# millecker/hadoop-1.0.3-gpu

Measured on AMD Instinct MI355X. Metric: K-Means job makespan + map-tasks/sec (whole node) at 1/2/4/8 MI355X, higher is better.
Workload: dtype fp32

## Files before the change

### hbmr/models/kmeans.py

```python
from __future__ import annotations

import base64
import logging
import math
import os
import threading
import time

import numpy as np
import torch

from ..gpu.splitjob import SplitJob, SplitSpec
from ..mapred import counters as C

log = logging.getLogger("hbmr.kmeans")

K_KEY = "hbmr.kmeans.k"
D_KEY = "hbmr.kmeans.dims"
INPUT_KEY = "hbmr.kmeans.input"
SPLIT_PTS_KEY = "hbmr.split.points"
CIN_KEY = "hbmr.kmeans.centroids.in"
COUT_KEY = "hbmr.kmeans.centroids.out"
INIT_KEY = "hbmr.kmeans.centroids.init"
NCENTERS_KEY = "hbmr.kmeans.synthetic.centers"
RETURN_KEY = "hbmr.kmeans.return.centroids"
CDIR_KEY = "hbmr.kmeans.centroids.dir"
EXACT_KEY = "hbmr.kmeans.exact"
EXACT_MFMA_KEY = "hbmr.kmeans.exact.mfma"
COMBINER_KEY = "hbmr.kmeans.combiner"
BOUNDS_KEY = "hbmr.kmeans.exact.bounds"

_M32 = 0xFFFFFFFF


def _mix32(x: torch.Tensor) -> torch.Tensor:
    x = x & _M32
    x = ((x ^ (x >> 16)) * 0x45D9F3B) & _M32
    x = ((x ^ (x >> 16)) * 0x45D9F3B) & _M32
    return x ^ (x >> 16)


def _uniform(c: torch.Tensor) -> torch.Tensor:
    return (_mix32(c).to(torch.float64) + 0.5) * (1.0 / 4294967296.0)


def _gauss(c1: torch.Tensor, c2: torch.Tensor) -> torch.Tensor:
    u1 = _uniform(c1)
    u2 = _uniform(c2)
    return torch.sqrt(-2.0 * torch.log(u1)) * torch.cos(2.0 * math.pi * u2)


def synthetic_points(seed: int, start: int, n: int, d: int, centers: int, device,
                     chunk: int = 1 << 18) -> torch.Tensor:
    dev = torch.device(device)
    out = torch.empty(n, d, dtype=torch.float32, device=dev)
    j = torch.arange(d, dtype=torch.int64, device=dev)
    cidx = torch.arange(centers, dtype=torch.int64, device=dev)
    s = (seed * 0x9E3779B1) & _M32
    cc = (cidx[:, None] * 131071 + j[None, :] + s * 7) & _M32
    cen = 10.0 * _gauss(cc * 2 + 1, cc * 2 + 2)
    for a in range(0, n, chunk):
        b = min(n, a + chunk)
        p = torch.arange(start + a, start + b, dtype=torch.int64, device=dev)
        lab = _mix32(p * 3 + s) % centers
        base = ((p[:, None] & 0xFFFFFF) * 1024 + j[None, :] + (s << 7)) & _M32
        noise = _gauss(base * 2 + 11, base * 2 + 12 + (p[:, None] >> 24))
        out[a:b] = (cen[lab] + noise).to(torch.float32)
    return out


def encode_centroids(c: torch.Tensor) -> str:
    a = c.detach().to("cpu", torch.float32).contiguous().numpy()
    return f"{a.shape[0]}x{a.shape[1]}:" + base64.b64encode(a.tobytes()).decode()


def decode_centroids(s: str) -> torch.Tensor:
    shp, b = s.split(":", 1)
    k, d = map(int, shp.split("x"))
    return torch.from_numpy(np.frombuffer(base64.b64decode(b), dtype=np.float32).copy()
                            ).reshape(k, d)


class CentroidStore:

    def __init__(self):
        self.lock = threading.Lock()
        self.host: dict[str, torch.Tensor] = {}
        self.images: dict[tuple, object] = {}
        self.order: list[str] = []
        self.keep = 4

    def put_host(self, key, cen):
        with self.lock:
            self.host[key] = cen
            for k in [k for k in self.images if k[0] == key]:
                self.images.pop(k)
            self._touch(key)

    def put_image(self, key, device, img):
        with self.lock:
            self.host.pop(key, None)
            self.images[(key, str(device))] = img
            self._touch(key)

    def _touch(self, key):
        if key in self.order:
            self.order.remove(key)
        self.order.append(key)
        while len(self.order) > self.keep:
            old = self.order.pop(0)
            self.host.pop(old, None)
            for k in [k for k in self.images if k[0] == old]:
                self.images.pop(k)
# ... 93 lines not shown
_BASELINES: "dict" = {}
_BASE_LOCK = threading.Lock()
_BASE_MAX = 4096


def _baseline_plan(ctxs, datas, k, dp, fx, exact, enabled):
    have, new, plain = [], [], []
    bases, keys = [], []
    seen = set()
    dev = str(ctxs[0].device)
    with _BASE_LOCK:
        for i, (c, d) in enumerate(zip(ctxs, datas)):
            sp = c.spec.split
            sk = sp.get("key") if enabled and isinstance(sp, dict) else None
            key = None if sk is None else (sk, dev, k, dp, fx, exact)
            keys.append(key)
            if key is None or key in seen:
                plain.append(i)
                bases.append(None)
                continue
            seen.add(key)
            b = _BASELINES.get(key)
            x = d.xb if exact else d
            if b is not None and b.data_ptr == x.data_ptr() and b.n == x.shape[0]:
                have.append(i)
                bases.append(b)
            else:
                new.append(i)
                bases.append(None)
    return have, new, plain, bases, keys


def _baseline_bytes(b) -> int:
    return sum(t.numel() * t.element_size() for t in (b.g, b.S0, b.N0, getattr(b, "gap", None))
               if t is not None)


def _drop_baselines(split_key, device):
    dev = f"cuda:{device}" if isinstance(device, int) else str(device)
    with _BASE_LOCK:
        for key in [kk for kk in _BASELINES if kk[0] == split_key and kk[1] == dev]:
            _BASELINES.pop(key)


def _install_baselines(entries, stream, cache=None, grown=None):
    ev = torch.cuda.Event()
    ev.record(stream)
    charge = []
    with _BASE_LOCK:
        for key, b in entries:
            b.event, b.stream = ev, stream
            old = _BASELINES.pop(key, None)
            _BASELINES[key] = b
            if old is not b:
                charge.append((key, b, _baseline_bytes(b)))
            elif grown and grown.get(id(b)):
                charge.append((key, b, grown[id(b)]))
        while len(_BASELINES) > _BASE_MAX:
            _BASELINES.pop(next(iter(_BASELINES)))
    if cache is not None and charge:
        cache.add_listener(_drop_baselines)
        idx = stream.device.index if stream is not None else 0
        for key, b, nbytes in charge:
            if not cache.charge(key[0], idx, nbytes):
                with _BASE_LOCK:
                    if _BASELINES.get(key) is b:
                        _BASELINES.pop(key)


def _exact_stats(cin, device):
    key = (cin, str(device))
    with _EXACT_LOCK:
        t = _EXACT_STATS.get(key)
        if t is None:
            t = _EXACT_STATS[key] = torch.zeros(3, dtype=torch.int64, device=device)
        return t


def _exact_skipped(cin, device):
    key = (cin, str(device))
    with _EXACT_LOCK:
        t = _EXACT_SKIPPED.get(key)
        if t is None:
            t = _EXACT_SKIPPED[key] = torch.zeros(1, dtype=torch.int64, device=device)
        return t


class KMeansSplitJob(SplitJob):
    collective_reduce = True
    needs_reduce = True

    def configure(self, conf):
        self.conf = conf
        self.k = conf.get_int(K_KEY, 64)
        self.d = conf.get_int(D_KEY, 128)
        self.input = conf.get(INPUT_KEY, "synthetic:100000:1")
        self.split_points = conf.get_int(SPLIT_PTS_KEY, 500_000)
        self.cin = conf.get(CIN_KEY)
        self.cout = conf.get(COUT_KEY)
        self.centers = conf.get_int(NCENTERS_KEY, self.k)
        self.fx_shift = conf.get_int("hbmr.kmeans.fx.shift", 24)
        self.cdir = conf.get(CDIR_KEY)
        self.exact = conf.get_boolean(EXACT_KEY, False)
        self.exact_dtype = torch.bfloat16 if (conf.get(EXACT_MFMA_KEY) or "f16").lower() in (
            "bf16", "bfloat16") else torch.float16
        self.bounds = conf.get_boolean(BOUNDS_KEY, True)
        self.combiner = (conf.get(COMBINER_KEY) or "delta").lower()
        if self.combiner not in ("delta", "sorted"):
            raise ValueError(f"{COMBINER_KEY} must be delta or sorted, not {self.combiner!r}")
        init = conf.get(INIT_KEY)
        if init and self.cin and STORE.host_centroids(self.cin) is None:
            STORE.put_host(self.cin, decode_centroids(init))
        if self.cin and self.cdir and STORE.host_centroids(self.cin) is None:
            path = _centroid_file(self.cdir, self.cin)
            if os.path.exists(path):
                STORE.put_host(self.cin, torch.from_numpy(np.load(path)))

    _split_memo: dict = {}

    def get_splits(self, conf, trackers):
        if self.input.startswith("synthetic:"):
            mk = (self.input, self.split_points, self.d, self.centers, tuple(trackers),
                  self.exact)
            got = KMeansSplitJob._split_memo.get(mk)
            if got is not None:
                return got
            if len(KMeansSplitJob._split_memo) > 16:
                KMeansSplitJob._split_memo.clear()
            out = KMeansSplitJob._split_memo[mk] = self._synthetic_splits(trackers)
            return out
        return self._file_splits(conf, trackers)

    def _synthetic_splits(self, trackers):
        _, n, seed = self.input.split(":")
        n, seed = int(n), int(seed)
        per = self.split_points
        nsplits = max(1, math.ceil(n / per))
        out = []
        for i in range(nsplits):
            a = i * per
            m = min(per, n - a)
            key = f"kmeans-syn:{seed}:{self.d}:{self.centers}:{a}:{m}" + \
                (":exact" if self.exact else "")
            loc = [trackers[i * len(trackers) // nsplits]] if trackers else []
            out.append(SplitSpec(i, key, "synthetic",
                                 {"seed": seed, "start": a, "n": m}, loc, m * self.d * 2))
        return out

    def _file_splits(self, conf, trackers):
        from ..mapred.formats import FileInputFormat, SequenceFileInputFormat
        from ..mapred.jobconf import JobConf
        jc = JobConf(conf)
        FileInputFormat.setInputPaths(jc, self.input)
        fmt = SequenceFileInputFormat()
        nmaps = max(1, conf.get_int("mapred.map.tasks", 1))
        if conf.get_long("mapred.min.split.size", 0) <= 1 and "://" not in self.input:
            total = sum(f.length for f in fmt.list_status(jc))
            jc.set_long("mapred.min.split.size", max(1, -(-total // nmaps)))
        splits = fmt.getSplits(jc, nmaps)
        out = []
        for i, s in enumerate(splits):
            key = f"kmeans-file:{s.path}:{s.start}:{s.length}" + (":exact" if self.exact else "")
            loc = [trackers[i % len(trackers)]] if trackers else []
            out.append(SplitSpec(i, key, "file", {"path": s.path, "start": s.start,
                                                  "length": s.length}, loc, s.length))
        return out

    def _load_raw(self, spec: SplitSpec, device):
        if spec.kind == "synthetic":
            p = spec.params
            return synthetic_points(p["seed"], p["start"], p["n"], self.d, self.centers, device)
        return self._load_file_split(spec.params, device)

    def _load_fp32(self, spec: SplitSpec, device):
        return self._load_raw(spec, device).to(torch.bfloat16)

    def split_nbytes(self, data) -> int:
        nb = getattr(data, "nbytes", None)
        if callable(nb):
            return int(nb())
        return super().split_nbytes(data)

    def load_split_host(self, spec: SplitSpec):
        if spec.kind != "file":
            return None
        from ..io import nativeio
        p = spec.params
        n = p["length"] // (20 + 4 * self.d) + 2
        host = torch.empty(n, self.d, dtype=torch.float32,
# ... 92 lines not shown
    def _map_gpu_batch(self, ctxs, datas):
        from ..ops import kmeans as km
        ctx = ctxs[0]
        img = STORE.image(self.cin, ctx.device)
        ready = getattr(img, "ready", None)
        if ready is not None:
            torch.cuda.current_stream().wait_event(ready)
        for t in (img.cbf, img.chalf):
            t.record_stream(torch.cuda.current_stream())
        B = len(datas)
        if self.exact:
            return self._map_exact(ctxs, datas, img)
        have, new, plain, bases, keys = _baseline_plan(
            ctxs, datas, self.k, img.dp, img.fx_shift, False, self.combiner == "delta")
        ws, labels = self._scratch(ctx, [d.shape[0] for d in datas], self.k)
        sums = torch.empty(B, self.k, img.dp, dtype=torch.int64, device=ctx.device)
        counts = torch.empty(B, self.k, dtype=torch.int64, device=ctx.device)
        order = have + new + plain
        H = len(have)
        S, N = sums.unbind(0), counts.unbind(0)
        out = [None] * B
        for j, i in enumerate(order):
            out[i] = (S[j], N[j])
        installed = []
        if have:
            hb = [bases[i] for i in have]
            km.map_batch_delta([datas[i] for i in have], img, sums[:H], counts[:H], labels, ws,
                               hb, stream=ctx.stream)
            for i, b in zip(have, hb):
                b.S0, b.N0 = out[i]
                installed.append((keys[i], b))
        rest = new + plain
        if rest:
            km.map_batch_gpu([datas[i] for i in rest], img, sums[H:], counts[H:], labels, ws,
                             stream=ctx.stream, zero_outputs=True)
            if new:
                total = sum(datas[i].shape[0] for i in rest)
                gall = labels[:total].clone()
                off = 0
                newset = set(new)
                for i in rest:
                    n = datas[i].shape[0]
                    if keys[i] is not None and i in newset:
                        installed.append((keys[i], km.Baseline(gall[off:off + n], *out[i],
                                                                datas[i].data_ptr(), n)))
                    off += n
        if installed:
            _install_baselines(installed, ctx.stream, getattr(ctx, "split_cache", None))
        for c, d in zip(ctxs, datas):
            c.reporter.incrCounter(C.TASK_GROUP, C.MAP_INPUT_RECORDS, d.shape[0])
        return out

    def _map_exact(self, ctxs, datas, img):
        from ..ops import kmeans as km
        from ..utils.trace import TRACE
        if TRACE.on:
            TRACE.instant("kmeans.map_exact", n=len(datas))
        ctx = ctxs[0]
        store = ctx.tracker.__dict__.setdefault("_scratch", {})
        scratch = store.setdefault(("kmeans-exact", str(ctx.device), id(ctx.stream)), {})
        stats = _exact_stats(self.cin, ctx.device)
        have, new, plain, bases, keys = _baseline_plan(
            ctxs, datas, self.k, img.dp, img.fx_shift, True, self.combiner == "delta")
        B = len(datas)
        sums = torch.empty(B, self.k, img.dp, dtype=torch.int64, device=ctx.device)
        counts = torch.empty(B, self.k, dtype=torch.int64, device=ctx.device)
        order = have + new + plain
        pos = {i: j for j, i in enumerate(order)}
        H = len(have)
        installed = []
        grown = None
        if have:
            ns = [datas[i].shape[0] for i in have]
            total = sum(ns)
            lab = scratch.get("labcat")
            if lab is None or lab.numel() < total:
                lab = scratch["labcat"] = torch.empty(total, dtype=torch.int32, device=ctx.device)
            need = km.delta_workspace_bytes(total, H, self.k)
            if scratch.get("dws") is None or scratch["dws"].numel() < need:
                scratch["dws"] = torch.empty(need, dtype=torch.uint8, device=ctx.device)
            hb = [bases[i] for i in have]
            bounded = self.bounds and self.combiner == "delta" and km.bounds_supported(img)
            if bounded:
                nogap = [b for b in hb if b.gap is None]
                km.assign_exact_batch([datas[i] for i in have], img, stats, lab, scratch,
                                      stream=ctx.stream, bounds=hb,
                                      skipped=_exact_skipped(self.cin, ctx.device))
                grown = {id(b): b.gap.numel() * b.gap.element_size() for b in nogap}
            else:
                km.assign_exact_batch([datas[i] for i in have], img, stats, lab, scratch,
                                      stream=ctx.stream)
            km.delta_combine([datas[i].x32 for i in have], lab, self.k, sums[:H], counts[:H],
                             scratch["dws"], hb, fx_shift=img.fx_shift, stream=ctx.stream,
                             keep_bounds=bounded)
            for i, b in zip(have, hb):
                b.S0, b.N0 = sums[pos[i]], counts[pos[i]]
                installed.append((keys[i], b))
        for i in new + plain:
            d = datas[i]
            s, c = sums[pos[i]], counts[pos[i]]
            s.zero_()
            c.zero_()
            lab = km.assign_exact(d, img, stats, scratch, stream=ctx.stream)
            need = km.workspace_bytes(d.shape[0], img.k)
            if scratch.get("ws") is None or scratch["ws"].numel() < need:
                scratch["ws"] = torch.empty(max(need, 1 << 20), dtype=torch.uint8,
                                            device=ctx.device)
            km.accumulate(d.x32, lab, img.k, s, c, fx_shift=img.fx_shift, stream=ctx.stream,
                          workspace=scratch["ws"])
            if keys[i] is not None and i in new:
                b = km.Baseline(lab.clone(), s, c, d.xb.data_ptr(), d.shape[0])
                installed.append((keys[i], b))
        if installed:
            _install_baselines(installed, ctx.stream, getattr(ctx, "split_cache", None), grown)
        for c, d in zip(ctxs, datas):
            c.reporter.incrCounter(C.TASK_GROUP, C.MAP_INPUT_RECORDS, d.shape[0])
        return [(sums[pos[i]], counts[pos[i]]) for i in range(B)]

    def map_cpu(self, ctx, points):
        from ..ops import kmeans as km
        cen = STORE.host_centroids(self.cin)
        if cen is None:
            raise KeyError(f"centroids {self.cin!r} not resident")
        sums, counts = km.new_partials(self.k, self.d, "cpu")
        st = [0]
        km.map_split_cpu(points, cen, sums, counts, nthreads=ctx.cpu_threads,
                         fx_shift=self.fx_shift, exact=self.exact, stats=st)
        if self.exact:
            ctx.reporter.incrCounter("KMEANS", "EXACT_FLAGGED_POINTS", st[0])
        ctx.reporter.incrCounter(C.TASK_GROUP, C.MAP_INPUT_RECORDS, points.shape[0])
        return sums, counts

    def map_sim(self, ctx, points):
        if points is None:
            ctx.reporter.incrCounter(C.TASK_GROUP, C.MAP_INPUT_RECORDS, 0)
            return None
        return self.map_cpu(ctx, points)

    def combine(self, ctx, outputs):
        from ..ops import kmeans as km
        dev = ctx.device if ctx.device is not None else torch.device("cpu")
        dp = km.padded_dim(self.d) if dev.type == "cuda" else self.d
        outputs = [o for o in outputs if o is not None]
        if dev.type == "cuda":
            cur = torch.cuda.current_stream()
            for s, c in outputs:
                if s.is_cuda:
                    s.record_stream(cur)
                    c.record_stream(cur)
        from ..utils.trace import TRACE
        if TRACE.on:
            TRACE.instant("kmeans.combine.recorded", n=len(outputs))
        same = [(s, c) for s, c in outputs if s.device == dev and s.shape[1] == dp]
        other = [(s, c) for s, c in outputs if not (s.device == dev and s.shape[1] == dp)]
        if same:
            sums, counts = _sum_slabs(same)
        else:
            sums = torch.zeros(self.k, dp, dtype=torch.int64, device=dev)
            counts = torch.zeros(self.k, dtype=torch.int64, device=dev)
        for s, c in other:
            sums[:, :s.shape[1]] += s.to(dev, non_blocking=True)
            counts += c.to(dev, non_blocking=True)
        return sums, counts

    def reduce(self, ctx, combined):
        from ..ops import kmeans as km
        from ..utils.trace import TRACE
        sums, counts = combined
        k, dp = sums.shape
        packed = torch.cat([sums.reshape(-1), counts])
        sim = getattr(ctx, "simulated_collective_s", None)
        with TRACE.span("kmeans.allreduce", nbytes=packed.numel() * 8):
            if sim is None:
                ctx.comm.all_reduce(packed)
            else:
                ctx.sim_ready = max(time.time(), getattr(ctx, "sim_base", 0.0)) + sim
        sums = packed[:k * dp].view(k, dp)
        counts = packed[k * dp:]
        est = _EXACT_STATS.pop((self.cin, str(sums.device)), None) \
            if self.exact and sums.device.type == "cuda" else None
        esk = _EXACT_SKIPPED.pop((self.cin, str(sums.device)), None) \
            if self.exact and sums.device.type == "cuda" else None
        killed = getattr(ctx, "killed", None)
        if killed is not None and killed():
            raise RuntimeError("reduce killed (collective restart): result not published")
        if sums.device.type == "cuda":
            old = STORE.image(self.cin, sums.device)
            ready = getattr(old, "ready", None)
            if ready is not None:
                torch.cuda.current_stream().wait_event(ready)
            img = km.CentroidImage.__new__(km.CentroidImage)
            img.__dict__.update(old.__dict__)
            img.cen = old.cen.clone()
            img.cbf = old.cbf.clone()
            img.chalf = old.chalf.clone()
            img.shift2 = torch.zeros_like(old.shift2)
            img.refresh(sums, counts)
            if self.exact:
                img.image16(self.exact_dtype)
                img.neighbors()
            img.ready = torch.cuda.Event()
            img.ready.record()
            host_cen = cen_ev = None
            if ctx.rank == 0 and (self.cdir or self.conf.get_boolean(RETURN_KEY, False)):
                host_cen = torch.empty(tuple(img.cen.shape), dtype=torch.float32,
                                       pin_memory=True)
                host_cen.copy_(img.cen, non_blocking=True)
                cen_ev = torch.cuda.Event()
                cen_ev.record()
            if TRACE.on:
                TRACE.instant("kmeans.refresh_launched")
            STORE.put_image(self.cout, sums.device, img)
            rel = getattr(ctx, "release_dependents", None)
            if rel is not None:
                rel()
            vals = [img.shift2.max().double().sqrt(), counts.sum().double()]
            if est is not None:
                vals += list(est.double().unbind(0))
            if esk is not None:
                vals.append(esk[0].double())
            got = torch.stack(vals).tolist()
            shift, npts = got[0], got[1]
            if esk is not None:
                ctx.reporter.incrCounter("KMEANS", "EXACT_BOUND_SKIPPED_POINTS", int(got[-1]))
            if est is not None:
                for name, v in zip(("EXACT_FLAGGED_POINTS", "EXACT_RELABELLED_POINTS",
                                    "EXACT_NEIGHBOUR_SCANS"), got[2:5]):
                    ctx.reporter.incrCounter("KMEANS", name, int(v))
            if TRACE.on:
                TRACE.instant("kmeans.shift_synced")
            new_cen = None
        else:
            host_cen = cen_ev = None
            old = STORE.host_centroids(self.cin)
            if sim is not None:
                new_cen, shift, npts = old, 0.0, 0
            else:
                cnt = counts.to(torch.float64)[:, None]
                s = sums[:, :self.d].to(torch.float64) / float(1 << self.fx_shift)
                new_cen = torch.where(cnt > 0, s / cnt.clamp(min=1),
                                      old.to(torch.float64)).to(torch.float32)
                shift = float((new_cen - old).norm(dim=1).max()) if self.k else 0.0
                npts = int(counts.sum().item())
            STORE.put_host(self.cout, new_cen)
            rel = getattr(ctx, "release_dependents", None)
            if rel is not None:
                rel()
            if sim is not None:
                delay = ctx.sim_ready - time.time()
                if delay > 0:
                    time.sleep(delay)
        self._write_output(ctx, counts, new_cen)
        if TRACE.on:
            TRACE.instant("kmeans.output_written")
        res = {"shift": shift, "points": int(npts), "centroids_key": self.cout}
        if host_cen is not None:
            cen_ev.synchronize()
        if ctx.rank == 0 and self.cdir:
            cen = new_cen if new_cen is not None else host_cen
            _save_centroids(self.cdir, self.cout, cen[:, :self.d])
        if ctx.rank == 0 and self.conf.get_boolean(RETURN_KEY, False):
            cen = new_cen if new_cen is not None else host_cen
            res["centroids"] = encode_centroids(cen[:, :self.d])
        if TRACE.on:
            TRACE.instant("kmeans.reduce_return")
        return res

    def poison_result(self, ctx):
        with STORE.lock:
            host = STORE.host.get(self.cout)
            if host is not None:
                STORE.host[self.cout] = host + 1.0
            for key, img in list(STORE.images.items()):
                if key[0] == self.cout:
                    STORE.images.pop(key)
                    STORE.host[self.cout] = img.cen.detach().to("cpu")[:, :self.d] + 1.0

    def _write_output(self, ctx, counts, new_cen):
        out = self.conf.get("mapred.output.dir")
        if not out:
            return
        import os

        from ..io import sequencefile as seqf
        from ..io.writable import FloatVectorWritable, IntWritable
        cen = new_cen if new_cen is not None else STORE.host_centroids(self.cout)
        W = ctx.world_size
        per = math.ceil(self.k / W)
        lo, hi = ctx.rank * per, min(self.k, (ctx.rank + 1) * per)
        os.makedirs(out, exist_ok=True)
        with seqf.Writer(os.path.join(out, f"part-{ctx.rank:05d}"), IntWritable,
                         FloatVectorWritable) as w:
            for j in range(lo, hi):
                w.append(IntWritable(j), FloatVectorWritable(cen[j].numpy()))


def make_iteration_conf(base, k, d, inp, split_points, cin, cout, init=None,
                        return_centroids=False):
    from ..mapred.jobconf import JobConf
    job = JobConf(base)
    job.set_job_name(f"kmeans {cin}->{cout}")
    job.set("hbmr.splitjob.class", "hbmr.models.kmeans:KMeansSplitJob")
    job.set("hbmr.gpu.mapper.class", "hbmr.models.kmeans:KMeansSplitJob")
    job.set_int(K_KEY, k)
    job.set_int(D_KEY, d)
    job.set(INPUT_KEY, inp)
    job.set_int(SPLIT_PTS_KEY, split_points)
# ... 189 lines not shown
```

### hbmr/ops/_lib.py

```python
from __future__ import annotations

import ctypes
import os
import threading
from pathlib import Path

import torch

_LIB_PATH = Path(__file__).resolve().parent.parent / "lib" / "libhbmr.so"
_lock = threading.Lock()
_lib = None

c_void_p = ctypes.c_void_p
c_long = ctypes.c_long
c_int = ctypes.c_int
c_uint = ctypes.c_uint
c_uint64 = ctypes.c_uint64
c_double_p = ctypes.POINTER(ctypes.c_double)

_SIGS = {
    "hbmr_kmeans_assign_bf16": (c_int, [c_void_p, c_long, c_int, c_void_p, c_void_p, c_int,
                                        c_void_p, c_void_p, c_void_p]),
    "hbmr_kmeans_accum_bf16": (c_int, [c_void_p, c_long, c_int, c_void_p, c_int, c_void_p,
                                       c_void_p, c_int, c_void_p, c_long, c_int, c_void_p]),
    "hbmr_kmeans_accum_f32": (c_int, [c_void_p, c_long, c_int, c_void_p, c_int, c_void_p,
                                      c_void_p, c_int, c_void_p, c_long, c_int, c_void_p]),
    "hbmr_kmeans_assign_top3_bf16": (c_int, [c_void_p, c_long, c_int, c_void_p, c_void_p, c_int,
                                             c_void_p, c_void_p, c_void_p, c_void_p, c_void_p]),
    "hbmr_kmeans_assign_top3_f16": (c_int, [c_void_p, c_long, c_int, c_void_p, c_void_p, c_int,
                                            c_void_p, c_void_p, c_void_p, c_void_p, c_void_p]),
    "hbmr_kmeans_exact_prep": (c_int, [c_void_p, c_long, c_int, c_int, c_int, c_int, c_void_p,
                                       c_void_p, c_void_p, c_void_p, c_void_p]),
    "hbmr_kmeans_assign_top3_q1_grouped": (c_int, [c_int, c_void_p, c_void_p, c_int, c_int,
                                                   c_void_p, c_void_p, c_void_p, c_int, c_void_p,
                                                   c_void_p, c_void_p, c_void_p, c_int, c_int,
                                                   c_void_p, c_void_p, c_void_p, c_void_p,
                                                   c_void_p, c_long, c_void_p, c_void_p]),
    "hbmr_kmeans_bound_workspace_bytes": (c_long, [c_long, c_int, c_int]),
    "hbmr_kmeans_assign_top3_q1_bounded": (c_int, [c_int, c_void_p, c_void_p, c_int, c_int,
                                                   c_void_p, c_void_p, c_int, c_void_p,
                                                   c_void_p, c_void_p, c_void_p, c_int, c_int,
                                                   c_void_p, c_void_p, c_void_p, c_void_p,
                                                   c_void_p, c_long, c_void_p,
                                                   c_void_p, c_void_p, c_void_p, c_void_p,
                                                   c_void_p, c_long, c_void_p, c_void_p]),
    "hbmr_kmeans_centroid_nbr": (c_int, [c_void_p, c_int, c_int, c_int, c_void_p, c_void_p,
                                         c_void_p, c_void_p]),
    "hbmr_kmeans_image16": (c_int, [c_void_p, c_int, c_int, c_int, c_int, c_int, c_void_p,
                                    c_void_p, c_void_p, c_void_p, c_void_p, c_void_p]),
    "hbmr_kmeans_image16_tiled": (c_int, [c_void_p, c_int, c_int, c_void_p, c_void_p]),
    "hbmr_kmeans_set_exact_kernel": (c_int, [c_int]),
    "hbmr_kmeans_get_exact_kernel": (c_int, []),
    "hbmr_kmeans_refine_f32": (c_int, [c_void_p, c_long, c_int, c_int, c_void_p, c_void_p,
                                       c_void_p, c_void_p, c_int, c_int, c_void_p, c_void_p,
                                       c_void_p, c_void_p, c_void_p, c_void_p, c_int, c_void_p,
                                       c_void_p, c_void_p, c_void_p, c_void_p, c_int,
                                       c_void_p]),
    "hbmr_kmeans_refine_batch_bytes": (c_long, [c_int, c_void_p]),
    "hbmr_kmeans_assign_top3_grouped": (c_int, [c_int, c_void_p, c_void_p, c_int, c_int,
                                                c_void_p, c_void_p, c_int, c_void_p, c_void_p,
                                                c_void_p, c_void_p, c_void_p]),
    "hbmr_kmeans_refine_batch_q1g": (c_int, [c_int, c_void_p, c_int, c_int, c_int, c_void_p,
                                             c_void_p, c_void_p, c_void_p, c_void_p, c_void_p,
                                             c_void_p, c_void_p, c_void_p, c_void_p, c_void_p,
                                             c_void_p, c_long, c_void_p, c_void_p]),
    "hbmr_kmeans_refine_batch_q1": (c_int, [c_int, c_void_p, c_int, c_int, c_int, c_int,
                                            c_void_p, c_void_p, c_void_p, c_void_p, c_void_p,
                                            c_void_p, c_void_p, c_void_p, c_void_p, c_void_p,
                                            c_void_p, c_void_p, c_void_p, c_long, c_int,
                                            c_void_p, c_void_p]),
    "hbmr_kmeans_refine_batch_finish": (c_int, [c_int, c_void_p, c_void_p, c_void_p, c_int,
                                                c_int, c_void_p, c_int, c_int, c_void_p,
                                                c_void_p, c_void_p, c_void_p, c_int, c_void_p,
                                                c_int, c_void_p, c_long, c_void_p]),
    "hbmr_kmeans_accum_workspace_bytes": (c_long, [c_long, c_int]),
    "hbmr_kmeans_batch_workspace_bytes": (c_long, [c_long, c_int, c_int]),
    "hbmr_kmeans_map_batch": (c_int, [c_int, c_void_p, c_void_p, c_int, c_void_p, c_void_p, c_int,
                                      c_int, c_void_p, c_void_p, c_long, c_void_p, c_void_p,
                                      c_int, c_int, c_void_p]),
    "hbmr_kmeans_delta_workspace_bytes": (c_long, [c_long, c_int, c_int]),
    "hbmr_kmeans_delta_combine": (c_int, [c_int, c_void_p, c_void_p, c_int, c_int, c_int,
                                          c_void_p, c_void_p, c_long, c_void_p, c_void_p, c_int,
                                          c_void_p, c_void_p, c_void_p, c_void_p]),
    "hbmr_kmeans_map_batch_delta": (c_int, [c_int, c_void_p, c_void_p, c_int, c_void_p, c_void_p,
                                            c_int, c_int, c_void_p, c_void_p, c_long, c_void_p,
                                            c_void_p, c_int, c_void_p, c_void_p, c_void_p,
                                            c_void_p]),
    "hbmr_kmeans_update": (c_int, [c_void_p, c_void_p, c_int, c_int, c_int, c_int, c_int,
                                   c_void_p, c_void_p, c_void_p, c_void_p, c_void_p]),
    "hbmr_kmeans_padded_k": (c_int, [c_int]),
    "hbmr_kmeans_map_cpu_f32": (c_int, [c_void_p, c_long, c_int, c_void_p, c_int, c_void_p,
                                        c_void_p, c_void_p, c_double_p, c_int, c_int]),
    "hbmr_kmeans_map_cpu_f32_ex": (c_int, [c_void_p, c_long, c_int, c_void_p, c_int, c_void_p,
                                           c_void_p, c_void_p, c_double_p, c_int, c_int, c_int,
                                           c_void_p]),
    "hbmr_kmeans_padded_dim": (c_int, [c_int]),
    "hbmr_f32_to_bf16_pad": (c_int, [c_void_p, c_long, c_int, c_int, c_void_p, c_void_p]),
    "hbmr_radix_sort_workspace_bytes": (c_long, [c_long]),
    "hbmr_radix_onesweep_workspace_bytes": (c_long, [c_long]),
    "hbmr_radix_onesweep_status_bytes": (c_long, [c_long]),
    "hbmr_radix_sort_keys_u64": (c_int, [c_void_p, c_void_p, c_long, c_int, c_int, c_void_p,
                                         c_long, c_void_p, c_long, c_void_p, c_void_p, c_int,
                                         c_void_p]),
    "hbmr_radix_sort_pairs_u64": (c_int, [c_void_p, c_void_p, c_void_p, c_void_p, c_long, c_int,
                                          c_int, c_void_p, c_long, c_void_p]),
    "hbmr_teragen": (c_int, [c_long, c_long, c_void_p, c_void_p]),
    "hbmr_tera_keys": (c_int, [c_void_p, c_long, c_int, c_void_p, c_void_p, c_void_p]),
    "hbmr_gather_u64": (c_int, [c_void_p, c_void_p, c_long, c_void_p, c_void_p]),
    "hbmr_gather_records": (c_int, [c_void_p, c_void_p, c_long, c_int, c_void_p, c_void_p]),
    "hbmr_split_offsets": (c_int, [c_void_p, c_void_p, c_long, c_void_p, c_void_p, c_int,
                                   c_void_p, c_void_p]),
    "hbmr_check_sorted": (c_int, [c_void_p, c_void_p, c_long, c_void_p, c_void_p]),
    "hbmr_tera_keys_part": (c_int, [c_void_p, c_long, c_int, c_void_p, c_void_p, c_int, c_void_p,
                                    c_void_p, c_void_p, c_void_p]),
    "hbmr_tera_collect": (c_int, [c_void_p, c_void_p, c_void_p, c_void_p, c_void_p, c_int, c_long,
                                  c_void_p, c_void_p, c_void_p, c_void_p, c_void_p]),
    "hbmr_tera_collect_slots": (c_int, [c_void_p, c_void_p, c_void_p, c_int, c_int, c_long,
                                        c_void_p, c_void_p, c_void_p]),
    "hbmr_gather_records_multi": (c_int, [c_void_p, c_void_p, c_void_p, c_void_p, c_long, c_int,
                                          c_void_p, c_void_p]),
    "hbmr_tera_partition_workspace_bytes": (c_long, [c_long, c_int]),
    "hbmr_tera_collect_gid": (c_int, [c_void_p, c_void_p, c_void_p, c_void_p, c_int, c_long,
                                      c_int, c_uint64, c_uint, c_uint, c_int, c_void_p, c_void_p,
                                      c_void_p]),
    "hbmr_gather_records_gid": (c_int, [c_void_p, c_void_p, c_void_p, c_long, c_int, c_void_p,
                                        c_void_p, c_void_p, c_void_p, c_void_p]),
    "hbmr_tera_group_stats": (c_int, [c_void_p, c_void_p, c_long, c_void_p, c_void_p, c_void_p,
                                      c_void_p]),
    "hbmr_radix_set_onesweep_waves": (c_int, [c_int]),
    "hbmr_gather_set_unroll": (c_int, [c_int]),
    "hbmr_tera_tie_fix_scratch_bytes": (c_long, [c_long, c_int]),
    "hbmr_tera_tie_fix_records": (c_int, [c_void_p, c_void_p, c_void_p, c_long, c_int, c_uint64,
                                          c_uint, c_uint, c_int, c_void_p, c_void_p, c_void_p,
                                          c_long, c_void_p]),
    "hbmr_merge_path": (c_int, [c_void_p, c_void_p, c_void_p, c_long, c_void_p, c_void_p, c_void_p,
                                c_long, c_void_p, c_void_p, c_void_p, c_void_p]),
    "hbmr_tera_tie_fix": (c_int, [c_void_p, c_void_p, c_void_p, c_long, c_void_p, c_void_p]),
    "hbmr_tera_partition": (c_int, [c_void_p, c_long, c_int, c_void_p, c_void_p, c_int, c_void_p,
                                    c_void_p, c_void_p, c_void_p, c_void_p, c_void_p, c_long,
                                    c_void_p]),
    "hbmr_wc_tiles": (c_long, [c_long]),
    "hbmr_wc_tokenize_count": (c_int, [c_void_p, c_long, c_void_p, c_void_p]),
    "hbmr_wc_tokenize_write": (c_int, [c_void_p, c_long, c_void_p, c_void_p, c_void_p, c_void_p]),
    "hbmr_wc_insert": (c_int, [c_void_p, c_long, c_void_p, c_void_p, c_void_p, c_long, c_void_p,
                               c_void_p, c_long, c_void_p, c_void_p]),
    "hbmr_wc_compact": (c_int, [c_void_p, c_long, c_void_p, c_void_p, c_long, c_int, c_void_p,
                                c_void_p, c_void_p, c_void_p, c_void_p, c_void_p]),
    "hbmr_wc_pack": (c_int, [c_void_p, c_void_p, c_void_p, c_void_p, c_long, c_void_p, c_void_p,
                             c_void_p]),
    "hbmr_grep_cand_count": (c_int, [c_void_p, c_long, c_void_p, c_void_p, c_int, c_int, c_int,
                                     c_int, c_void_p, c_void_p, c_void_p]),
    "hbmr_grep_cand_write": (c_int, [c_void_p, c_long, c_void_p, c_void_p, c_int, c_int, c_int,
                                     c_int, c_void_p, c_void_p, c_void_p, c_void_p, c_void_p]),
    "hbmr_grep_select_blocks": (c_long, [c_long]),
    "hbmr_grep_block_max": (c_int, [c_void_p, c_long, c_void_p, c_void_p]),
    "hbmr_grep_prefix_max": (c_int, [c_void_p, c_long, c_void_p, c_void_p, c_void_p]),
    "hbmr_grep_select_count": (c_int, [c_void_p, c_void_p, c_void_p, c_long, c_void_p, c_void_p]),
# ... 88 lines not shown
```

### hbmr/ops/kmeans.py

```python
from __future__ import annotations

import ctypes
import os
import threading

import torch

from . import _lib
from ..utils.trace import TRACE

SUPPORTED_DP = (64, 128, 256)


def _nullctx():
    import contextlib
    return contextlib.nullcontext()
FX_SHIFT = 24
NBR_L = 256


def padded_dim(d: int) -> int:
    for dp in SUPPORTED_DP:
        if d <= dp:
            return dp
# ... 236 lines not shown
            _lib.check(rc, "hbmr_kmeans_exact_prep")
            return
        x64 = self.x32.double()
        self.xnorm = x64.norm(dim=1).float()
        lim = 65504.0 if dtype == torch.float16 else float("inf")
        xb = self.x32.clamp(-lim, lim).to(dtype)
        xb64 = xb.double()
        self.xbn2 = xb64.pow(2).sum(1).float()
        self.xerr = _f32_up((x64 - xb64).norm(dim=1))
        self.xb = xb.contiguous()

    @property
    def shape(self):
        return self.xb.shape

    def nbytes(self) -> int:
        return sum(t.numel() * t.element_size() for t in (self.xb, self.x32, self.xnorm,
                                                          self.xbn2, self.xerr))


def assign_top3(points: torch.Tensor, img: CentroidImage, labels, cand, scores, margin,
                stream=None) -> None:
    n, dp = points.shape
    if points.dtype not in (torch.bfloat16, torch.float16) or dp != img.dp or \
            not points.is_contiguous():
        raise ValueError("points must be contiguous bf16/fp16 [n, dp] matching the image")
    for t, dt, m in ((labels, torch.int32, 1), (cand, torch.int32, 2), (scores, torch.float32, 1),
                     (margin, torch.float32, 2)):
        if t.numel() != m * n or t.dtype != dt or not t.is_contiguous():
            raise ValueError("top-3 outputs: labels/scores [n], cand/margin [2n]")
    f16 = points.dtype == torch.float16
    with torch.cuda.stream(stream) if stream is not None else _nullctx():
        c16, ch = img.image16(points.dtype)[:2]
    fn = "hbmr_kmeans_assign_top3_f16" if f16 else "hbmr_kmeans_assign_top3_bf16"
    rc = getattr(_lib.load(), fn)(
        _ptr(points), n, dp, _ptr(c16), _ptr(ch), img.k_pad, _ptr(labels),
        _ptr(cand), _ptr(scores), _ptr(margin), _lib.stream_handle(stream))
    _lib.check(rc, fn)


REFINE_VERSION = int(os.environ.get("HBMR_REFINE", "3"))
MAX_REFINE_BATCH = 64


def _refine_ws(ns: list, device, scratch: dict | None):
    arr = (ctypes.c_long * len(ns))(*ns)
    need = int(_lib.load().hbmr_kmeans_refine_batch_bytes(len(ns), arr))
    if need < 0:
        raise ValueError("refine batch of 1..64 splits expected")
    ws = None if scratch is None else scratch.get("refine_ws")
    if ws is None or ws.numel() < need:
        ws = torch.empty(need, dtype=torch.uint8, device=device)
        if scratch is not None:
            scratch["refine_ws"] = ws
    return arr, ws


class _RefineBatch:

    def __init__(self, splits: list, img: "CentroidImage", stats, scratch, stream):
        self.splits, self.img, self.stats, self.stream = splits, img, stats, stream
        self.dt = splits[0].xb.dtype
        self.ns, self.ws = _refine_ws([sp.shape[0] for sp in splits], splits[0].x32.device,
                                      scratch)
        with torch.cuda.stream(stream) if stream is not None else _nullctx():
            self.norms = img.norms(self.dt)
            self.nbr = img.neighbors()
            self.pd = img.pair_dist()
        self.labels = [None] * len(splits)
        self.lib = _lib.load()
        self.st = _lib.stream_handle(stream)

    def q1(self, i, labels_ptr, cand, scores, margin):
        sp, img = self.splits[i], self.img
        cn, cmax, ce, cemax = self.norms
        self.labels[i] = labels_ptr
        rc = self.lib.hbmr_kmeans_refine_batch_q1(
            len(self.splits), self.ns, i, img.d, img.k, img.k_pad, _ptr(sp.xnorm),
            _ptr(sp.xbn2), _ptr(sp.xerr), _ptr(cn), _ptr(cmax), _ptr(ce), _ptr(cemax),
            labels_ptr, _ptr(cand), _ptr(scores), _ptr(margin), _ptr(self.stats),
            _ptr(self.ws), self.ws.numel(), int(i == 0), _ptr(self.pd), self.st)
        _lib.check(rc, "hbmr_kmeans_refine_batch_q1")

    def finish(self):
        B = len(self.splits)
        img = self.img
        _, cmax, _, cemax = self.norms
        ni, nd, L = self.nbr
        xs = (ctypes.c_void_p * B)(*[sp.x32.data_ptr() for sp in self.splits])
        ls = (ctypes.c_void_p * B)(*[(lp.value if isinstance(lp, ctypes.c_void_p) else lp)
                                     for lp in self.labels])
        rc = self.lib.hbmr_kmeans_refine_batch_finish(
            B, self.ns, xs, ls, img.d, self.splits[0].x32.shape[1], _ptr(img.cen), img.k,
            img.k_pad, _ptr(cmax), _ptr(cemax), _ptr(ni), _ptr(nd), L, _ptr(self.stats),
            self.stats.numel(), _ptr(self.ws), self.ws.numel(), self.st)
        _lib.check(rc, "hbmr_kmeans_refine_batch_finish")


def refine_f32(split: ExactSplit, img: CentroidImage, labels, cand, scores, margin,
               stats: torch.Tensor, stream=None, scratch: dict | None = None) -> None:
    n = split.shape[0]
    if stats.dtype != torch.int64 or stats.numel() < 3:
        raise ValueError("stats must be int64 [3]")
    if labels.numel() != n or cand.numel() != 2 * n or margin.numel() != 2 * n:
        raise ValueError("labels [n], cand/margin [2n] from assign_top3 expected")
    if REFINE_VERSION >= 3:
        rb = _RefineBatch([split], img, stats, scratch, stream)
        rb.q1(0, labels.data_ptr(), cand, scores, margin)
        rb.finish()
        return
    with torch.cuda.stream(stream) if stream is not None else _nullctx():
        cn, cmax, ce, cemax = img.norms(split.xb.dtype)
        ni, nd, L = img.neighbors()
    rc = _lib.load().hbmr_kmeans_refine_f32(
        _ptr(split.x32), n, img.d, split.x32.shape[1], _ptr(split.xnorm), _ptr(split.xbn2),
        _ptr(split.xerr), _ptr(img.cen), img.k, img.k_pad, _ptr(cn), _ptr(cmax), _ptr(ce),
        _ptr(cemax), _ptr(ni), _ptr(nd), L,
        _ptr(labels), _ptr(cand), _ptr(scores), _ptr(margin), _ptr(stats), stats.numel(),
        _lib.stream_handle(stream))
    _lib.check(rc, "hbmr_kmeans_refine_f32")


def assign_exact(split: ExactSplit, img: CentroidImage, stats: torch.Tensor,
                 scratch: dict | None = None, stream=None) -> torch.Tensor:
    n = split.shape[0]
    dev = split.xb.device
    scratch = {} if scratch is None else scratch
    key = ("exact", n)
    bufs = scratch.get(key)
    if bufs is None:
        bufs = scratch[key] = (torch.empty(n, dtype=torch.int32, device=dev),
                               torch.empty(2 * n, dtype=torch.int32, device=dev),
                               torch.empty(n, dtype=torch.float32, device=dev),
                               torch.empty(2 * n, dtype=torch.float32, device=dev))
    lab, cand, sc, mg = bufs
    assign_top3(split.xb, img, lab, cand, sc, mg, stream=stream)
    refine_f32(split, img, lab, cand, sc, mg, stats, stream=stream, scratch=scratch)
    return lab


def bounds_supported(img: CentroidImage) -> bool:
    return REFINE_VERSION >= 3 and img.dp <= 128 and GROUPED_EXACT and FUSED_Q1 and \
        img.cen.is_cuda and _lib.load().hbmr_kmeans_get_exact_kernel() == 3


def assign_exact_batch(splits: list, img: CentroidImage, stats: torch.Tensor, out: torch.Tensor,
                       scratch: dict | None = None, stream=None, bounds: list | None = None,
                       skipped: torch.Tensor | None = None) -> None:
    if not splits:
        return
    if bounds is not None and (len(bounds) != len(splits) or not bounds_supported(img)):
        raise ValueError("bounds: one baseline per split, grouped fused v3 assign (dp <= 128)")
    dev = splits[0].xb.device
    total = sum(sp.shape[0] for sp in splits)
    if out.dtype != torch.int32 or out.numel() < total or not out.is_contiguous():
        raise ValueError("out must be contiguous int32 with room for every split's labels")
    if stats.dtype != torch.int64 or stats.numel() < 3:
        raise ValueError("stats must be int64 [3]")
    dt = splits[0].xb.dtype
    for sp in splits:
        if sp.xb.dtype != dt or dt not in (torch.bfloat16, torch.float16) or \
                sp.xb.shape[1] != img.dp or not sp.xb.is_contiguous() or \
                not sp.x32.is_contiguous():
            raise ValueError("exact splits must hold contiguous [n, dp] rows of one 16-bit type")
    nmax = max(sp.shape[0] for sp in splits)
    scratch = {} if scratch is None else scratch
    key = ("exact-batch", nmax)
    bufs = scratch.get(key)
    if bufs is None:
        for kk in [kk for kk in scratch if isinstance(kk, tuple) and kk[0] == "exact-batch"]:
            del scratch[kk]
        bufs = scratch[key] = (torch.empty(2 * nmax, dtype=torch.int32, device=dev),
                               torch.empty(nmax, dtype=torch.float32, device=dev),
                               torch.empty(2 * nmax, dtype=torch.float32, device=dev))
    cand, sc, mg = bufs
    grouped = REFINE_VERSION >= 3 and img.dp <= 128 and GROUPED_EXACT
    with torch.cuda.stream(stream) if stream is not None else _nullctx():
        c16, ch, cn, cmax, ce, cemax = img.image16(dt)
        ni, nd, L = (None, None, 0) if grouped else img.neighbors()
        newref = None
        if bounds is not None:
            img.cen.record_stream(torch.cuda.current_stream())
            newref = img.cen.clone()
    lib = _lib.load()
    top3 = lib.hbmr_kmeans_assign_top3_f16 if dt == torch.float16 else \
        lib.hbmr_kmeans_assign_top3_bf16
    st = _lib.stream_handle(stream)
    pc, ps, pm, pst = _ptr(cand), _ptr(sc), _ptr(mg), _ptr(stats)
    pcn, pcmax, pce, pcemax, pni, pnd = (_ptr(t) for t in (cn, cmax, ce, cemax, ni, nd))
    base, off = out.data_ptr(), 0
    for g0 in range(0, len(splits), MAX_REFINE_BATCH):
        group = splits[g0:g0 + MAX_REFINE_BATCH]
        if grouped:
            off += _exact_group(group, img, stats, base + 4 * off, c16, ch, (cn, cmax, ce, cemax),
                                dt, scratch, stream, lib, st,
                                None if bounds is None else bounds[g0:g0 + MAX_REFINE_BATCH],
                                skipped, newref)
            continue
        rb = _RefineBatch(group, img, stats, scratch, stream) if REFINE_VERSION >= 3 else None
        for i, sp in enumerate(group):
            n = sp.shape[0]
            pl = ctypes.c_void_p(base + 4 * off)
            rc = top3(_ptr(sp.xb), n, img.dp, _ptr(c16), _ptr(ch), img.k_pad, pl, pc, ps, pm, st)
            _lib.check(rc, "hbmr_kmeans_assign_top3")
            if rb is not None:
                rb.q1(i, pl, cand, sc, mg)
            else:
                rc = lib.hbmr_kmeans_refine_f32(
                    _ptr(sp.x32), n, img.d, sp.x32.shape[1], _ptr(sp.xnorm), _ptr(sp.xbn2),
                    _ptr(sp.xerr), _ptr(img.cen), img.k, img.k_pad, pcn, pcmax, pce, pcemax,
                    pni, pnd, L, pl, pc, ps, pm, pst, stats.numel(), st)
                _lib.check(rc, "hbmr_kmeans_refine_f32")
            off += n
        if rb is not None:
            rb.finish()


PAIR_DIST_MAX_K = int(os.environ.get("HBMR_PAIR_DIST_MAX_K", "8192"))
NBR_NATIVE_MAX_K = int(os.environ.get("HBMR_NBR_NATIVE_MAX_K", "8192"))
GROUPED_EXACT = os.environ.get("HBMR_EXACT_GROUPED", "1") != "0"
FUSED_Q1 = os.environ.get("HBMR_EXACT_FUSED_Q1", "1") != "0"


def _bounded_group(group, bases, img, labels_ptr, ch, norms, dt, scratch, stream, lib, st, rb,
                   skipped, newref):
    B = len(group)
    ns = [sp.shape[0] for sp in group]
    N = sum(ns)
    dev = group[0].xb.device
    cur = torch.cuda.current_stream() if stream is None else stream
    with torch.cuda.stream(cur):
        events, blocks = {}, {}
        for b in bases:
            if b.event is not None and b.stream is not None and b.stream != cur:
                events[id(b.event)] = b.event
        for ev in events.values():
            cur.wait_event(ev)
        for b in bases:
            if b.gap is None:
                b.gap, b.ref = torch.empty(b.g.numel(), dtype=torch.float32, device=dev), None
        for b, n in zip(bases, ns):
            if b.g.numel() != n or b.gap.numel() != n or \
                    (b.ref is not None and (tuple(b.ref.shape) != tuple(img.cen.shape) or
                                            not b.ref.is_contiguous())):
                raise ValueError("bounds: baseline does not match its split / the centroids")
            for t in (b.g, b.gap, b.ref):
                if t is not None:
                    base = t._base if t._base is not None else t
                    blocks[id(base)] = base
        for t in blocks.values():
            t.record_stream(cur)
        need = int(lib.hbmr_kmeans_bound_workspace_bytes(N, B, img.k))
        bws = scratch.get("bound_ws")
        if bws is None or bws.numel() < need:
            bws = scratch["bound_ws"] = torch.empty(need, dtype=torch.uint8, device=dev)
    P = ctypes.c_void_p * B
    cn, cmax, ce, cemax = norms
    refs = [b.ref for b in bases]
    for b in bases:
        b.ref = b.pending = None
    rc = lib.hbmr_kmeans_assign_top3_q1_bounded(
        B, P(*[sp.xb.data_ptr() for sp in group]), (ctypes.c_long * B)(*ns), img.dp,
        int(dt == torch.float16), _ptr(img.image16_tiled(dt)), _ptr(ch), img.k_pad, labels_ptr,
        P(*[sp.xnorm.data_ptr() for sp in group]), P(*[sp.xbn2.data_ptr() for sp in group]),
        P(*[sp.xerr.data_ptr() for sp in group]), img.d, img.k, _ptr(cn), _ptr(cmax), _ptr(ce),
        _ptr(cemax), _ptr(rb.ws), rb.ws.numel(), _ptr(rb.pd),
        P(*[b.g.data_ptr() for b in bases]), P(*[b.gap.data_ptr() for b in bases]),
        P(*[None if r is None else r.data_ptr() for r in refs]), _ptr(img.cen),
        _ptr(bws), bws.numel(), _ptr(skipped), st)
    _lib.check(rc, "hbmr_kmeans_assign_top3_q1_bounded")
    for b in bases:
        b.pending = newref


def _exact_group(group, img, stats, labels_ptr, c16, ch, norms, dt, scratch, stream, lib, st,
                 bases=None, skipped=None, newref=None):
    B = len(group)
    ns = [sp.shape[0] for sp in group]
    N = sum(ns)
    dev = group[0].xb.device
    P = ctypes.c_void_p * B
    xs = P(*[sp.xb.data_ptr() for sp in group])
    nsa = (ctypes.c_long * B)(*ns)
    if bases is not None:
        rb = _RefineBatch(group, img, stats, scratch, stream)
        if TRACE.on:
            TRACE.instant("kmeans.top3_launch", n=B)
        _bounded_group(group, bases, img, labels_ptr, ch, norms, dt, scratch, stream, lib, st, rb,
                       skipped, newref)
        o = 0
        for i in range(B):
            rb.labels[i] = labels_ptr + 4 * o
            o += ns[i]
        rb.finish()
        return N
    if FUSED_Q1 and img.dp <= 128:
        rb = _RefineBatch(group, img, stats, scratch, stream)
        if TRACE.on:
            TRACE.instant("kmeans.top3_launch", n=B)
        cn, cmax, ce, cemax = norms
        rc = lib.hbmr_kmeans_assign_top3_q1_grouped(
            B, xs, nsa, img.dp, int(dt == torch.float16), _ptr(c16),
            _ptr(img.image16_tiled(dt)), _ptr(ch), img.k_pad,
            labels_ptr, P(*[sp.xnorm.data_ptr() for sp in group]),
            P(*[sp.xbn2.data_ptr() for sp in group]), P(*[sp.xerr.data_ptr() for sp in group]),
            img.d, img.k, _ptr(cn), _ptr(cmax), _ptr(ce), _ptr(cemax), _ptr(rb.ws),
            rb.ws.numel(), _ptr(rb.pd), st)
        _lib.check(rc, "hbmr_kmeans_assign_top3_q1_grouped")
        o = 0
        for i in range(B):
            rb.labels[i] = labels_ptr + 4 * o
            o += ns[i]
        rb.finish()
        return N
    key = ("exact-group", N)
    bufs = scratch.get(key)
    if bufs is None:
        for kk in [kk for kk in scratch if isinstance(kk, tuple) and kk[0] == "exact-group"]:
            del scratch[kk]
        bufs = scratch[key] = (torch.empty(2 * N, dtype=torch.int32, device=dev),
                               torch.empty(N, dtype=torch.float32, device=dev),
                               torch.empty(2 * N, dtype=torch.float32, device=dev))
    cand, sc, mg = bufs
    rc = lib.hbmr_kmeans_assign_top3_grouped(B, xs, nsa, img.dp, int(dt == torch.float16),
                                             _ptr(c16), _ptr(ch), img.k_pad, labels_ptr,
                                             _ptr(cand), _ptr(sc), _ptr(mg), st)
    _lib.check(rc, "hbmr_kmeans_assign_top3_grouped")
    rb = _RefineBatch(group, img, stats, scratch, stream)
    cn, cmax, ce, cemax = norms
    rc = lib.hbmr_kmeans_refine_batch_q1g(
        B, nsa, img.d, img.k, img.k_pad, P(*[sp.xnorm.data_ptr() for sp in group]),
        P(*[sp.xbn2.data_ptr() for sp in group]), P(*[sp.xerr.data_ptr() for sp in group]),
        _ptr(cn), _ptr(cmax), _ptr(ce), _ptr(cemax), labels_ptr, _ptr(cand), _ptr(sc), _ptr(mg),
        _ptr(rb.ws), rb.ws.numel(), _ptr(rb.pd), st)
    _lib.check(rc, "hbmr_kmeans_refine_batch_q1g")
    o = 0
    for i in range(B):
        rb.labels[i] = labels_ptr + 4 * o
        o += ns[i]
    rb.finish()
    return N


def map_split_exact(split: ExactSplit, img: CentroidImage, sums, counts, scratch: dict,
                    stats: torch.Tensor, stream=None) -> None:
    n = split.shape[0]
    lab = assign_exact(split, img, stats, scratch, stream=stream)
    need = workspace_bytes(n, img.k)
    if scratch.get("ws") is None or scratch["ws"].numel() < need:
        scratch["ws"] = torch.empty(max(need, 1 << 20), dtype=torch.uint8, device=split.xb.device)
    accumulate(split.x32, lab, img.k, sums, counts, fx_shift=img.fx_shift, stream=stream,
               workspace=scratch["ws"])


def map_batch_gpu(splits: list, img: CentroidImage, sums: torch.Tensor, counts: torch.Tensor,
                  labels: torch.Tensor, workspace: torch.Tensor, stream=None,
                  zero_outputs: bool = True) -> None:
    B = len(splits)
    if B == 0:
        return
    for s in splits:
        if s.dtype != torch.bfloat16 or s.shape[1] != img.dp or not s.is_contiguous():
            raise ValueError("splits must be contiguous bf16 [n, dp]")
    if sums.shape != (B, img.k, img.dp) or counts.shape != (B, img.k):
        raise ValueError("batch output shape mismatch")
    need_lab, need_ws = batch_scratch_sizes([s.shape[0] for s in splits], img.k)
    if labels.numel() < need_lab:
        raise ValueError("labels scratch too small")
    lib = _lib.load()
    if workspace.numel() < need_ws:
        raise ValueError("workspace too small")
    ptrs = (ctypes.c_void_p * B)(*[s.data_ptr() for s in splits])
    ns = (ctypes.c_long * B)(*[s.shape[0] for s in splits])
    rc = lib.hbmr_kmeans_map_batch(B, ptrs, ns, img.dp, _ptr(img.cbf), _ptr(img.chalf), img.k_pad,
                                   img.k, _ptr(labels), _ptr(workspace), workspace.numel(),
                                   _ptr(sums), _ptr(counts), img.fx_shift, int(zero_outputs),
                                   _lib.stream_handle(stream))
    _lib.check(rc, "hbmr_kmeans_map_batch")


class Baseline:
    __slots__ = ("g", "S0", "N0", "event", "stream", "data_ptr", "n", "gap", "ref", "pending")

    def __init__(self, g, S0, N0, data_ptr, n):
        self.g, self.S0, self.N0 = g, S0, N0
        self.gap = self.ref = self.pending = None
        self.event = None
        self.stream = None
        self.data_ptr, self.n = data_ptr, n

    def labels_advanced(self, bounded: bool = False) -> None:
        self.ref = self.pending if bounded else None
        self.pending = None


def delta_workspace_bytes(total: int, ntasks: int, k: int) -> int:
    return int(_lib.load().hbmr_kmeans_delta_workspace_bytes(total, ntasks, k))


def _delta_args(xs, bases, stream):
    B = len(xs)
    st = torch.cuda.current_stream() if stream is None else stream
    events, blocks = {}, {}
    for b in bases:
        if b.event is not None and b.stream is not None and b.stream != st:
            events[id(b.event)] = b.event
        for t in (b.g, b.S0, b.N0):
            base = t._base if t._base is not None else t
            blocks[id(base)] = base
    for ev in events.values():
        st.wait_event(ev)
    for t in blocks.values():
        t.record_stream(st)
    ptrs = (ctypes.c_void_p * B)(*[x.data_ptr() for x in xs])
    ns = (ctypes.c_long * B)(*[x.shape[0] for x in xs])
    gs = (ctypes.c_void_p * B)(*[b.g.data_ptr() for b in bases])
    s0 = (ctypes.c_void_p * B)(*[b.S0.data_ptr() for b in bases])
    n0 = (ctypes.c_void_p * B)(*[b.N0.data_ptr() for b in bases])
    return ptrs, ns, gs, s0, n0


def map_batch_delta(splits: list, img: CentroidImage, sums: torch.Tensor, counts: torch.Tensor,
                    labels: torch.Tensor, workspace: torch.Tensor, bases: list,
                    stream=None) -> None:
    B = len(splits)
    if B == 0:
        return
    if B > 64 or len(bases) != B:
        raise ValueError("at most 64 splits per delta batch, one baseline each")
    for s, b in zip(splits, bases):
        if s.dtype != torch.bfloat16 or s.shape[1] != img.dp or not s.is_contiguous():
            raise ValueError("splits must be contiguous bf16 [n, dp]")
        if b.g.numel() != s.shape[0] or tuple(b.S0.shape) != (img.k, img.dp) or \
                b.N0.numel() != img.k:
            raise ValueError("baseline does not match its split")
    if sums.shape != (B, img.k, img.dp) or counts.shape != (B, img.k) or \
            not sums.is_contiguous() or not counts.is_contiguous():
        raise ValueError("batch output shape mismatch")
    total = sum(s.shape[0] for s in splits)
    if labels.numel() < total:
        raise ValueError("labels scratch too small")
    need = delta_workspace_bytes(total, B, img.k)
    if workspace.numel() < need:
        raise ValueError("workspace too small")
    ptrs, ns, gs, s0, n0 = _delta_args(splits, bases, stream)
    for b in bases:
        b.labels_advanced()
    rc = _lib.load().hbmr_kmeans_map_batch_delta(
        B, ptrs, ns, img.dp, _ptr(img.cbf), _ptr(img.chalf), img.k_pad, img.k, _ptr(labels),
        _ptr(workspace), workspace.numel(), _ptr(sums), _ptr(counts), img.fx_shift, gs, s0, n0,
        _lib.stream_handle(stream))
    _lib.check(rc, "hbmr_kmeans_map_batch_delta")


def delta_combine(xs: list, labels: torch.Tensor, k: int, sums: torch.Tensor,
                  counts: torch.Tensor, workspace: torch.Tensor, bases: list,
                  fx_shift: int = FX_SHIFT, stream=None, keep_bounds: bool = False) -> None:
    B = len(xs)
    if B == 0:
        return
    pend = [b.pending for b in bases]
    for b in bases:
        b.labels_advanced()
    dp = xs[0].shape[1]
    f32 = xs[0].dtype == torch.float32
    for x, b in zip(xs, bases):
        if x.dtype != xs[0].dtype or x.shape[1] != dp or not x.is_contiguous() or \
                b.g.numel() != x.shape[0]:
            raise ValueError("delta_combine: rows/baselines mismatch")
# ... 47 lines not shown
```

### native/include/hbmr/hbmr.h

```cpp
#pragma once
#include <stddef.h>
#include <stdint.h>

#ifdef __cplusplus
extern "C" {
#endif

typedef struct ihipStream_t* hbmr_stream_t;

#ifndef HBMR_NO_HIP_DECLS
#include <hip/hip_runtime_api.h>
int hbmr_kmeans_assign_bf16(const void* X, long n, int dp, const void* C, const float* chalf,
                            int k_pad, int32_t* labels, float* scores, hipStream_t st);
int hbmr_kmeans_accum_bf16(const void* X, long n, int dp, const int32_t* labels, int k,
                           long long* sums, long long* counts, int fx_shift, void* ws,
                           long ws_bytes, int mode, hipStream_t st);
int hbmr_kmeans_accum_f32(const float* X, long n, int dp, const int32_t* labels, int k,
                          long long* sums, long long* counts, int fx_shift, void* ws,
                          long ws_bytes, int mode, hipStream_t st);
int hbmr_kmeans_assign_top3_bf16(const void* X, long n, int dp, const void* C, const float* chalf,
                                 int k_pad, int32_t* labels, int32_t* cand, float* scores,
                                 float* margin, hipStream_t st);
int hbmr_kmeans_assign_top3_f16(const void* X, long n, int dp, const void* C, const float* chalf,
                                int k_pad, int32_t* labels, int32_t* cand, float* scores,
                                float* margin, hipStream_t st);
int hbmr_kmeans_exact_prep(const float* x, long n, int d, int ldx, int dp, int f16, void* x16,
                           float* xnorm, float* xn2, float* xerr, hipStream_t st);
int hbmr_kmeans_centroid_nbr(const float* cen, int k, int d, int L, int32_t* di, float* dv,
                             float* pd, hipStream_t st);
int hbmr_kmeans_image16(const float* cen, int k, int d, int dp, int k_pad, int f16, void* c16,
                        float* chalf, float* cnorm, float* cerr, float* maxima, hipStream_t st);
int hbmr_kmeans_image16_tiled(const void* c16, int k_pad, int dp, void* c16t, hipStream_t st);
int hbmr_kmeans_set_stamps(void* p);
int hbmr_kmeans_refine_f32(const float* X32, long n, int d, int ldx, const float* xnorm,
                           const float* xbn2, const float* xerr, const float* C32, int k,
                           int k_pad, const float* cnorm, const float* cmax, const float* cerr,
                           const float* cerrmax, const int32_t* nbr_idx,
                           const float* nbr_dist, int L, int32_t* labels, const int32_t* cand,
                           const float* scores, const float* margin, unsigned long long* stats,
                           int nstats, hipStream_t st);
int hbmr_kmeans_assign_top3_q1_grouped(int nsplit, const void* const* X, const long* n, int dp,
                                       int f16, const void* C, const void* Ct,
                                       const float* chalf, int k_pad,
                                       int32_t* labels, const float* const* xnorm,
                                       const float* const* xbn2, const float* const* xerr,
                                       int d, int k, const float* cnorm, const float* cmax,
                                       const float* cerr, const float* cerrmax, void* ws,
                                       long ws_bytes, const float* dcc, hipStream_t st);
long hbmr_kmeans_bound_workspace_bytes(long total, int nsplit, int k);
int hbmr_kmeans_assign_top3_q1_bounded(int nsplit, const void* const* X, const long* n, int dp,
                                       int f16, const void* Ct, const float* chalf, int k_pad,
                                       int32_t* labels, const float* const* xnorm,
                                       const float* const* xbn2, const float* const* xerr,
                                       int d, int k, const float* cnorm, const float* cmax,
                                       const float* cerr, const float* cerrmax, void* ws,
                                       long ws_bytes, const float* dcc,
                                       const int32_t* const* g, float* const* gap,
                                       const float* const* ref, const float* cen, void* bws,
                                       long bws_bytes, unsigned long long* skipped,
                                       hipStream_t st);
int hbmr_kmeans_assign_top3_grouped(int nsplit, const void* const* X, const long* n, int dp,
                                    int f16, const void* C, const float* chalf, int k_pad,
                                    int32_t* labels, int32_t* cand, float* scores, float* margin,
                                    hipStream_t st);
int hbmr_kmeans_refine_batch_q1g(int nsplit, const long* ns, int d, int k, int k_pad,
                                 const float* const* xnorm, const float* const* xbn2,
                                 const float* const* xerr, const float* cnorm, const float* cmax,
                                 const float* cerr, const float* cerrmax, const int32_t* labels,
                                 const int32_t* cand, const float* scores, const float* margin,
                                 void* ws, long ws_bytes, const float* dcc, hipStream_t st);
long hbmr_kmeans_refine_batch_bytes(int nsplit, const long* ns);
int hbmr_kmeans_refine_batch_q1(int nsplit, const long* ns, int s, int d, int k, int k_pad,
                                const float* xnorm, const float* xbn2, const float* xerr,
                                const float* cnorm, const float* cmax, const float* cerr,
                                const float* cerrmax, const int32_t* labels, const int32_t* cand,
                                const float* scores, const float* margin,
                                unsigned long long* stats, void* ws, long ws_bytes, int reset,
                                const float* dcc, hipStream_t st);
int hbmr_kmeans_refine_batch_finish(int nsplit, const long* ns, const float* const* x32,
                                    int32_t* const* labels, int d, int ldx, const float* C32,
                                    int k, int k_pad, const float* cmax, const float* cerrmax,
                                    const int32_t* nbr_idx, const float* nbr_dist, int L,
                                    unsigned long long* stats, int nstats, void* ws,
                                    long ws_bytes, hipStream_t st);
int hbmr_kmeans_update(const long long* sums, const long long* counts, int fx_shift, int k, int d,
                       int dp, int k_pad, float* cen, void* cbf, float* chalf, float* shift2,
                       hipStream_t st);
int hbmr_kmeans_map_batch(int ntasks, const void* const* X, const long* n, int dp,
                          const void* C, const float* chalf, int k_pad, int k, int32_t* labels,
                          void* ws, long ws_bytes, long long* sums, long long* counts,
                          int fx_shift, int zero_outputs, hipStream_t st);
int hbmr_f32_to_bf16_pad(const float* src, long n, int d, int dp, void* dst, hipStream_t st);
#endif
int hbmr_kmeans_padded_dim(int d);

#ifndef HBMR_NO_HIP_DECLS
int hbmr_radix_sort_pairs_u64(uint64_t* keys, uint32_t* vals, uint64_t* tkeys, uint32_t* tvals,
                              long n, int begin_bit, int end_bit, void* ws, long ws_bytes,
                              hipStream_t st);
int hbmr_teragen(long first_row, long nrows, void* out, hipStream_t st);
int hbmr_tera_keys(const void* records, long n, int stride, uint64_t* hi, uint64_t* lo,
                   hipStream_t st);
int hbmr_gather_u64(const uint64_t* src, const uint32_t* perm, long n, uint64_t* dst,
                    hipStream_t st);
int hbmr_gather_records(const void* src, const uint32_t* perm, long n, int record_bytes, void* dst,
                        hipStream_t st);
int hbmr_split_offsets(const uint64_t* hi, const uint64_t* lo, long n, const uint64_t* shi,
                       const uint64_t* slo, int nparts, long* offsets, hipStream_t st);
int hbmr_check_sorted(const uint64_t* hi, const uint64_t* lo, long n, unsigned long long* bad,
                      hipStream_t st);
int hbmr_tera_keys_part(const void* records, long n, int stride, const uint64_t* shi,
                        const uint64_t* slo, int nsplit, uint64_t* hi, uint64_t* lo,
                        uint64_t* pid, hipStream_t st);
int hbmr_tera_collect(const uint64_t* const* his, const uint64_t* const* los,
                      const uint32_t* const* rows, const long* starts, const long* prefix, int S,
                      long n, uint64_t* ohi, uint64_t* olo, uint32_t* osplit, uint32_t* orow,
                      hipStream_t st);
int hbmr_tera_collect_slots(const uint32_t* const* rows, const long* starts, const long* pre,
                            int S, int W, long C, uint32_t* osplit, uint32_t* orow,
                            hipStream_t st);
int hbmr_gather_records_multi(const void* const* bases, const uint32_t* split, const uint32_t* row,
                              const uint32_t* perm, long n, int record_bytes, void* dst,
                              hipStream_t st);
int hbmr_tera_collect_gid(const uint64_t* const* his, const uint32_t* const* rows,
                          const long* starts, const long* prefix, int S, long n, int pack,
                          uint64_t vlo, unsigned int m, unsigned int R, int sh, uint64_t* ohi,
                          uint32_t* ogid, hipStream_t st);
int hbmr_gather_records_gid(const void* const* bases, const uint32_t* gid, const uint64_t* packed,
                            long n, int record_bytes, void* dst, uint64_t* hi, uint64_t* lo,
                            uint32_t* win, hipStream_t st);
long hbmr_radix_onesweep_workspace_bytes(long n);
long hbmr_radix_onesweep_status_bytes(long n);
int hbmr_radix_sort_keys_u64(uint64_t* keys, uint64_t* tkeys, long n, int begin_bit, int end_bit,
                             void* ws, long ws_bytes, void* status, long status_bytes,
                             unsigned int* epoch, uint32_t* err, int copy_back, hipStream_t st);
long hbmr_tera_tie_fix_scratch_bytes(long cap, int record_bytes);
int hbmr_tera_group_stats(const uint64_t* hi, const uint64_t* lo, long n, const uint64_t* ph,
                          const uint64_t* pl, unsigned long long* acc, hipStream_t st);
int hbmr_tera_tie_fix_records(uint64_t* hi, uint64_t* lo, void* rec, long n, int record_bytes,
                              uint64_t vlo, unsigned int m, unsigned int R, int sh,
                              const uint32_t* win, unsigned int* flag, void* scratch, long cap,
                              hipStream_t st);
int hbmr_merge_path(const uint64_t* ahi, const uint64_t* alo, const uint32_t* av, long na,
                    const uint64_t* bhi, const uint64_t* blo, const uint32_t* bv, long nb,
                    uint64_t* ohi, uint64_t* olo, uint32_t* ov, hipStream_t st);
int hbmr_tera_tie_fix(const uint64_t* hi, uint64_t* lo, uint32_t* perm, long n,
                      unsigned int* flag, hipStream_t st);
int hbmr_tera_partition(const void* records, long n, int stride, const uint64_t* shi,
                        const uint64_t* slo, int nsplit, uint64_t* ohi, uint64_t* olo,
                        uint32_t* orow, long* offsets, unsigned long long* kmm, void* ws,
                        long ws_bytes, hipStream_t st);
#endif
long hbmr_radix_sort_workspace_bytes(long n);
long hbmr_tera_partition_workspace_bytes(long n, int nparts);

#ifndef HBMR_NO_HIP_DECLS
int hbmr_gemm_bf16_tn(const void* A, const void* Bt, void* C, long M, long N, long K, float alpha,
                      int out_bf16, hipStream_t st);
int hbmr_gemm_bf16_tn_ex(const void* A, const void* Bt, void* C, long M, long N, long K,
                         float alpha, int out_bf16, double* partials, hipStream_t st);
#endif
#ifndef HBMR_NO_HIP_DECLS
long hbmr_wc_tiles(long n);
int hbmr_wc_tokenize_count(const uint8_t* buf, long n, uint32_t* tile_counts, hipStream_t st);
int hbmr_wc_tokenize_write(const uint8_t* buf, long n, const long* tile_base, uint32_t* starts,
                           uint32_t* lens, hipStream_t st);
int hbmr_wc_insert(const uint8_t* buf, long n, const uint32_t* starts, const uint32_t* lens,
// ... 72 lines not shown
```

### native/kernels/kmeans.hip

```cpp
#include "common.h"
#include "../include/hbmr/hbmr.h"
#include <algorithm>
#include <cstdlib>
#include <cstring>
#include <type_traits>

namespace {

constexpr int kWaves = 4;
constexpr int kThreads = kWaves * HBMR_WAVE;
constexpr int kCK = 64;

template <bool F16>
__device__ __forceinline__ f32x16 mfma32x32x16(bf16x8 a, bf16x8 b, f32x16 c) {
  if constexpr (F16)
    return __builtin_amdgcn_mfma_f32_32x32x16_f16(__builtin_bit_cast(f16x8, a),
                                                  __builtin_bit_cast(f16x8, b), c, 0, 0, 0);
  else
    return __builtin_amdgcn_mfma_f32_32x32x16_bf16(a, b, c, 0, 0, 0);
}

template <int D> struct AssignCfg {
  static constexpr int KS = D / 16;
  static constexpr int CPR = D / 8;
// ... 1953 lines not shown
  const int q = w / 32, r = w % 32;
  c16t[P] = c16[(T * 32 + r) * cpr + q];
}

__global__ __launch_bounds__(128) void kmeans_image16_kernel(
    const float* __restrict__ cen, int k, int d, int dp, int f16, uint16_t* __restrict__ c16,
    float* __restrict__ chalf, float* __restrict__ cnorm, float* __restrict__ cerr,
    unsigned* __restrict__ maxbits) {
  const int j = blockIdx.x;
  const int tid = threadIdx.x;
  __shared__ float red[128];
  __shared__ double red64[2][128];
  float nrm = 0.f;
  double a = 0.0, e = 0.0;
  for (int i = tid; i < dp; i += 128) {
    const float v = (j < k && i < d) ? cen[(size_t)j * d + i] : 0.f;
    const uint16_t b = f16 ? hbmr_f32_to_f16_sat(v) : hbmr_f32_to_bf16(v);
    const float vt = f16 ? hbmr_f16_to_f32(b) : hbmr_bf16_to_f32(b);
    c16[(size_t)j * dp + i] = b;
    nrm += vt * vt;
    a = fma((double)v, (double)v, a);
    const double df = (double)v - (double)vt;
    e = fma(df, df, e);
  }
  red[tid] = nrm;
  red64[0][tid] = a;
  red64[1][tid] = e;
  __syncthreads();
  for (int s = 64; s > 0; s >>= 1) {
    if (tid < s) {
      red[tid] += red[tid + s];
      red64[0][tid] += red64[0][tid + s];
      red64[1][tid] += red64[1][tid + s];
    }
    __syncthreads();
  }
  if (tid == 0) {
    chalf[j] = j < k ? -0.5f * red[0] : -1.0e30f;
    if (j < k) {
      const float cn = __double2float_ru(sqrt(red64[0][0]) * (1.0 + 0x1p-50));
      const float ce = __double2float_ru(sqrt(red64[1][0]) * (1.0 + 0x1p-50));
      cnorm[j] = cn;
      cerr[j] = ce;
      atomicMax(maxbits + 0, __float_as_uint(cn));
      atomicMax(maxbits + 1, __float_as_uint(ce));
    }
  }
}

struct ExactQ1 {
  uint32_t row, split;
  int32_t b, s, t;
  float sb, m3, x2, xn, xe, pad0, pad1;
};
struct ExactQ2 {
  uint32_t row, split;
  int32_t w, pad;
  double dw;
};
static_assert(sizeof(ExactQ1) == 48 && sizeof(ExactQ2) == 24, "queue entry layout");

constexpr int kQShards = 8;
constexpr int kQ1Per = 4;
constexpr int kQ2Lanes = 8;
constexpr int kQ2Per = HBMR_WAVE / kQ2Lanes;
constexpr int kRefineGrid = 2048;
inline long refine_grid() {
  static const long g = [] {
    const char* e = getenv("HBMR_REFINE_GRID");
    const long v = e ? atol(e) : 0;
    return v > 0 ? v : (long)kRefineGrid;
  }();
  return g;
}
constexpr int kStatsOff = 64;
constexpr int kRefineHdr = 512;
constexpr int kHdrClear = kStatsOff + kQShards * 4 * 8;

struct RefineTable {
  int nsplit;
  const float* x32[kMaxGroup];
  int32_t* labels[kMaxGroup];
};

__host__ __device__ inline long ceil_div(long a, long b) { return (a + b - 1) / b; }

struct RefineLayout {
  long cap1, cap2;
  unsigned g2;
  size_t off1, off2, bytes;
};
inline RefineLayout refine_layout(int nsplit, const long* ns) {
  RefineLayout L;
  long total = 0, cap1 = 0, nb_fused = 0;
  for (int i = 0; i < nsplit; ++i) {
    total += ns[i];
    cap1 += ceil_div(ceil_div(ns[i], 256 * kQ1Per), kQShards) * 256 * kQ1Per;
    nb_fused += ceil_div(ns[i], 256);
  }
  L.cap1 = std::max<long>(cap1, ceil_div(nb_fused, kQShards) * 256);
  L.g2 = (unsigned)std::max<long>(1, std::min<long>(refine_grid(), ceil_div(total, 4 * kQ2Per)));
  const long per_iter = (long)L.g2 * 4 * kQ2Per;
  L.cap2 = ceil_div(L.g2, kQShards) * 4 * kQ2Per * std::max<long>(1, ceil_div(total, per_iter));
  L.off1 = kRefineHdr;
  L.off2 = L.off1 + ((kQShards * (size_t)L.cap1 * sizeof(ExactQ1) + 255) & ~(size_t)255);
  L.bytes = L.off2 + kQShards * (size_t)L.cap2 * sizeof(ExactQ2);
  return L;
}

__device__ __forceinline__ long shard_slot(const uint32_t (&c)[kQShards], long cap, uint32_t i) {
  uint32_t acc = 0;
  long slot = 0;
#pragma unroll
  for (int j = 0; j < kQShards; ++j) {
    if (i >= acc && i < acc + c[j]) slot = (long)j * cap + (i - acc);
    acc += c[j];
  }
  return slot;
}

__device__ __forceinline__ uint32_t lane_rank(unsigned long long m) {
  return __builtin_amdgcn_mbcnt_hi((uint32_t)(m >> 32), __builtin_amdgcn_mbcnt_lo((uint32_t)m, 0u));
}

template <bool GAP>
__device__ __forceinline__ bool q1_certify(const ExactQ1& e, float m2, float cnb, float ceb, int k,
                                           double gam, double cm, double cem, double pack_rel,
                                           const float* __restrict__ cnorm,
                                           const float* __restrict__ cerr,
                                           const float* __restrict__ dcc, float& gap) {
  const double inflate = 1.0 + 0x1p-20;
  const double xn = ((double)e.xn + (double)e.xe) * inflate;
  const double x2 = (double)e.x2;
  const double sb = e.sb;
  const double mm = m2;
  const double amax = ((double)e.xe + cem) * inflate;
  double eb, es, dl_b, dl_s;
  exact_bound(sb, ((double)cnb + (double)ceb) * inflate, xn, x2,
              ((double)e.xe + (double)ceb) * inflate, gam, pack_rel, eb, dl_b);
  exact_bound(sb - mm, cm, xn, x2, amax, gam, pack_rel, es, dl_s);
  bool flag = !(mm > eb + es && dl_s >= 2.0 * amax);
  double marg = mm - (eb + es);
  const int b = e.b, sc = e.s, t = e.t;
  if (flag && dcc != nullptr && t < k && t != b) {
    const double ex = (double)e.xe * inflate;
    const double ebb = (double)ceb * inflate;
    const double ess = (double)cerr[sc] * inflate;
    const double dbs = ((double)dcc[(size_t)b * k + sc] + (double)ceb + (double)cerr[sc]) *
                       inflate;
    double eap_b, rb, eap_s, rs;
    score_err(sb, ((double)cnb + (double)ceb) * inflate, xn, x2, gam, pack_rel, eap_b, rb);
    score_err(sb - mm, ((double)cnorm[sc] + (double)cerr[sc]) * inflate, xn, x2, gam,
              pack_rel, eap_s, rs);
    const double ep = dbs * ex + rs * ess + rb * ebb + 0.5 * (ex + ebb) * (ex + ebb) +
                      eap_b + eap_s;
    double et, dl_t;
    const double m3 = e.m3;
    exact_bound(sb - m3, cm, xn, x2, amax, gam, pack_rel, et, dl_t);
    if (mm > ep && m3 > eb + et && dl_t >= 2.0 * amax) {
      flag = false;
      if constexpr (GAP) marg = fmin(mm - ep, m3 - (eb + et));
    }
  }
  if constexpr (GAP) {
    gap = 0.f;
    if (!flag && marg > 0.0) {
// ... 75 lines not shown
  __syncthreads();
  if (tid == 0) {
    uint32_t tot = 0;
#pragma unroll
    for (int w = 0; w < 4; ++w)
#pragma unroll
      for (int i = 0; i < kQ1Per; ++i) {
        const uint32_t c = wcnt[w][i];
        wcnt[w][i] = tot;
        tot += c;
      }
    base_s = tot ? atomicAdd(qcount + shard, tot) : 0u;
    if (tot) atomicAdd(stats + 4 * shard, (unsigned long long)tot);
  }
  __syncthreads();
  ExactQ1* out = q1 + (long)shard * cap1 + base_s;
#pragma unroll
  for (int i = 0; i < kQ1Per; ++i)
    if (flag[i]) out[wcnt[wave][i] + rank[i]] = e[i];
}

__global__ __launch_bounds__(256) void kmeans_refine_q1_kernel(
    long n, int sidx, int d, int k, const float* __restrict__ xnorm,
    const float* __restrict__ xbn2, const float* __restrict__ xerr,
    const float* __restrict__ cnorm, const float* __restrict__ cmax,
    const float* __restrict__ cerr, const float* __restrict__ cerrmax, double pack_rel,
    const int32_t* __restrict__ labels, const int32_t* __restrict__ cand,
    const float* __restrict__ score, const float* __restrict__ margin,
    uint32_t* __restrict__ qcount, ExactQ1* __restrict__ q1, long cap1,
    unsigned long long* __restrict__ stats, const float* __restrict__ dcc) {
  refine_q1_block(n, sidx, blockIdx.x, d, k, xnorm, xbn2, xerr, cnorm, cmax, cerr, cerrmax,
                  pack_rel, labels, cand, score, margin, n, qcount, q1, cap1, stats, dcc);
}

struct Q1Table {
  int nsplit;
  long total;
  long n[kMaxGroup];
  long off[kMaxGroup];
  long blk[kMaxGroup + 1];
  const float* xnorm[kMaxGroup];
  const float* xbn2[kMaxGroup];
  const float* xerr[kMaxGroup];
};

__global__ __launch_bounds__(256) void kmeans_refine_q1_grouped_kernel(
    const Q1Table tbl, int d, int k, const float* __restrict__ cnorm,
    const float* __restrict__ cmax, const float* __restrict__ cerr,
    const float* __restrict__ cerrmax, double pack_rel, const int32_t* __restrict__ labels,
    const int32_t* __restrict__ cand, const float* __restrict__ score,
    const float* __restrict__ margin, uint32_t* __restrict__ qcount, ExactQ1* __restrict__ q1,
    long cap1, unsigned long long* __restrict__ stats, const float* __restrict__ dcc) {
  const long b = blockIdx.x;
  int lo = 0, hi = tbl.nsplit;
  while (hi - lo > 1) {
    const int mid = (lo + hi) >> 1;
    if (tbl.blk[mid] <= b) lo = mid; else hi = mid;
  }
  const int s = __builtin_amdgcn_readfirstlane(lo);
  const long o = tbl.off[s];
  refine_q1_block(tbl.n[s], s, b - tbl.blk[s], d, k, tbl.xnorm[s], tbl.xbn2[s], tbl.xerr[s],
                  cnorm, cmax, cerr, cerrmax, pack_rel, labels + o, cand + o, score + o,
                  margin + o, tbl.total, qcount, q1, cap1, stats, dcc);
}

struct FusedQ1Fin {
  const float* xnorm;
  const float* xbn2;
  const float* xerr;
  int sidx;
  int k;
  double gam, pack_rel;
  const float* cmax_p;
  const float* cerrmax_p;
  const float* cnorm;
  const float* cerr;
  const float* dcc;
  uint32_t* qcount;
  ExactQ1* q1;
  long cap1;
  unsigned long long* stats;
  const uint32_t* idx;
  float* gap;

  template <class AM, int PB, bool BND = false>
  __device__ __forceinline__ void operator()(const AM (&am)[PB], int h, long p0, int col, long n,
                                             int32_t* __restrict__ labels) const {
    const int tid = threadIdx.x, lane = tid & 63, wave = tid >> 6;
    __shared__ uint32_t fq_cnt[4 * PB];
    __shared__ uint32_t fq_base;
    const int shard = blockIdx.x % kQShards;
    const double inflate = 1.0 + 0x1p-20;
    const double cem = (double)cerrmax_p[0] * inflate;
    const double cm = (double)cmax_p[0] * inflate + cem;
    ExactQ1 e[PB];
    bool flag[PB];
    uint32_t rank[PB];
#pragma unroll
    for (int pb = 0; pb < PB; ++pb) {
      float v[3];
      int c[3];
      am[pb].top3(v[0], v[1], v[2]);
#pragma unroll
      for (int i = 0; i < 3; ++i) c[i] = am[pb].cluster(v[i], h);
      float ov[3];
      int oc[3];
#pragma unroll
      for (int i = 0; i < 3; ++i) {
        ov[i] = __shfl_xor(v[i], 32);
        oc[i] = __shfl_xor(c[i], 32);
      }
#pragma unroll
      for (int i = 0; i < 3; ++i) insert3(v, c, ov[i], oc[i]);
      if constexpr (HasTracks<AM>::value) {
        if (((c[0] ^ c[1]) & AM::TMASK) == 0) {
          v[2] = v[0];
          c[2] = c[0];
        }
      }
      const long p = p0 + pb * 32 + col;
      flag[pb] = false;
      if (h == 0 && p < n) {
        long row = p;
        if constexpr (BND) row = idx[p];
        labels[row] = c[0];
        const float bs = am[pb].score(v[0]);
        const float m2 = bs - am[pb].score(v[1]);
        ExactQ1& q = e[pb];
        q.row = (uint32_t)row;
        q.split = (uint32_t)sidx;
        q.b = c[0];
        q.s = c[1];
        q.t = c[2];
        q.sb = bs;
        q.m3 = bs - am[pb].score(v[2]);
        q.x2 = xbn2[row];
        q.xn = xnorm[row];
        q.xe = xerr[row];
        q.pad0 = q.pad1 = 0.f;
        if constexpr (BND) {
          float gp = 0.f;
          flag[pb] = q.s < k && q1_certify<true>(q, m2, cnorm[q.b], cerr[q.b], k, gam, cm, cem,
                                                 pack_rel, cnorm, cerr, dcc, gp);
          gap[row] = gp;
        } else {
          flag[pb] = q.s < k && q1_flagged(q, m2, cnorm[q.b], cerr[q.b], k, gam, cm, cem,
                                           pack_rel, cnorm, cerr, dcc);
        }
      }
      const unsigned long long m = __ballot(flag[pb]);
      rank[pb] = lane_rank(m);
      if (lane == 0) fq_cnt[wave * PB + pb] = (uint32_t)__popcll(m);
    }
    __syncthreads();
    if (tid == 0) {
      uint32_t tot = 0;
#pragma unroll
      for (int i = 0; i < 4 * PB; ++i) {
        const uint32_t c = fq_cnt[i];
        fq_cnt[i] = tot;
        tot += c;
      }
      fq_base = tot ? atomicAdd(qcount + shard, tot) : 0u;
      if (tot) atomicAdd(stats + 4 * shard, (unsigned long long)tot);
    }
    __syncthreads();
    ExactQ1* out = q1 + (long)shard * cap1 + fq_base;
#pragma unroll
    for (int pb = 0; pb < PB; ++pb)
      if (flag[pb]) out[fq_cnt[wave * PB + pb] + rank[pb]] = e[pb];
  }
};

template <int D>
__device__ __forceinline__ void stage_tile32t(char* buf, const __bf16* __restrict__ Ct,
                                              const float* __restrict__ chalf, int tile, int wave,
                                              int lane) {
  using V = AssignV2<D>;
  const uint32_t loff = (uint32_t)lane * 16u;
#pragma unroll
  for (int i = 0; i < V::P; ++i) {
    const int base = (i * V::WAVES + wave) * HBMR_WAVE;
    const char* g = reinterpret_cast<const char*>(Ct) + (size_t)tile * V::TILE_BYTES +
                    (size_t)base * 16;
    __builtin_amdgcn_global_load_lds((const void*)(g + loff), (void*)(buf + base * 16), 16, 0, 0);
  }
  if (wave == 0 && lane < 32) {
    const char* g = reinterpret_cast<const char*>(chalf + (size_t)tile * 32);
    __builtin_amdgcn_global_load_lds((const void*)(g + loff / 4u), (void*)(buf + V::TILE_BYTES),
                                     4, 0, 0);
  }
}

__device__ __forceinline__ void tile_codes(uint32_t top, int t, uint32_t (&code)[16]) {
  const uint32_t base = top - ((uint32_t)t << 4);
#pragma unroll
  for (int r = 0; r < 16; ++r) {
    code[r] = base | (15u - r);
    asm("" : "+s"(code[r]));
  }
}

__device__ __forceinline__ void top2_insert(PackedTop2x8& am, const f32x16& acc,
                                            const uint32_t (&code)[16], uint32_t vmask) {
  constexpr int NT = PackedTop2x8::NT;
#pragma unroll
  for (int r = 0; r < 16; ++r) {
    if ((r / NT) % 2) continue;
    const float u = __uint_as_float((__float_as_uint(acc[r]) & vmask) | code[r]);
    const float v = __uint_as_float((__float_as_uint(acc[r + NT]) & vmask) | code[r + NT]);
    const float m = vmed3(am.tb[r % NT], u, v);
    am.ts[r % NT] = vmax3(m, am.ts[r % NT], am.ts[r % NT]);
    am.tb[r % NT] = vmax3(am.tb[r % NT], u, v);
  }
}

template <int D, bool F16, bool BND = false>
__device__ __forceinline__ void assign_tile_v3(const __bf16* __restrict__ X, long n,
                                               const __bf16* __restrict__ Ct,
                                               const float* __restrict__ chalf, int ntiles,
                                               int32_t* __restrict__ labels, long blk, char* smem,
                                               const FusedQ1Fin& fin) {
  static_assert(D <= 128, "v3 keeps two 32-point blocks of D <= 128 in registers");
  constexpr int PB = 2, NS = 4;
  using V = AssignV2<D, NS>;
  static_assert(V::WAVES == 4, "v3: 4 waves per workgroup");
  constexpr int KS = V::KS;
// ... 58 lines not shown
  int slot = 0;
  for (int t = 0; t < ntiles; ++t) {
    wait_tile_dmas<V::P, NS - 2>(max(0, min(NS - 2, ntiles - 2 - t)), w0);
    asm volatile("s_waitcnt lgkmcnt(0)" ::: "memory");
    __syncthreads();
    char* rbuf = smem + slot * V::BUF;
    if (t + NS < ntiles) stage_tile32t<D>(rbuf, Ct, chalf, t + NS, wave, lane);
    slot = slot + 1 == NS ? 0 : slot + 1;
    const char* nbuf = smem + slot * V::BUF;
    const char* nrow = nbuf + rowoff;
    f32x16 acc[PB];
#pragma unroll
    for (int s = 0; s < KS; ++s) {
#pragma unroll
      for (int pb = 0; pb < PB; ++pb)
        acc[pb] = mfma32x32x16<F16>(a[s], bfrag[pb][s], s == 0 ? bz : acc[pb]);
      a[s] = frag(nrow, s);
    }
    uint32_t code[16];
    tile_codes(top, t, code);
#pragma unroll
    for (int pb = 0; pb < PB; ++pb) top2_insert(am[pb], acc[pb], code, vmask);
    bias(nbuf, bz);
  }
  fin.template operator()<PackedTop2x8, PB, BND>(am, h, p0, col, n, labels);
}

struct TopQ1Table {
  int nsplit;
  const __bf16* X[kMaxGroup];
  const float* xnorm[kMaxGroup];
  const float* xbn2[kMaxGroup];
  const float* xerr[kMaxGroup];
  long off[kMaxGroup + 1];
  long blk[kMaxGroup + 1];
};

template <int D, bool F16>
__global__ __launch_bounds__(AssignV2<D>::THREADS, HBMR_EXACT_MINB) void
kmeans_assign_top3_q1_grouped_kernel(const TopQ1Table tbl, const __bf16* __restrict__ C,
                                     const float* __restrict__ chalf, int ntiles,
                                     int32_t* __restrict__ labels, FusedQ1Fin fin) {
  extern __shared__ __attribute__((aligned(16))) char smem[];
  const long b = hbmr_xcd_remap(blockIdx.x, gridDim.x);
  int lo = 0, hi = tbl.nsplit;
  while (hi - lo > 1) {
    const int mid = (lo + hi) >> 1;
    if (tbl.blk[mid] <= b) lo = mid; else hi = mid;
  }
  const int s = __builtin_amdgcn_readfirstlane(lo);
  const long o = tbl.off[s];
  fin.xnorm = tbl.xnorm[s];
  fin.xbn2 = tbl.xbn2[s];
  fin.xerr = tbl.xerr[s];
  fin.sidx = s;
  assign_tile_v2<D, 2, true, F16, false, FusedQ1Fin>(
      tbl.X[s], tbl.off[s + 1] - o, C, chalf,
                                                     ntiles, labels + o, nullptr, b - tbl.blk[s],
                                                     smem, nullptr, nullptr, -1, &fin);
}

template <int D, bool F16>
__global__ __launch_bounds__(256, HBMR_EXACT_MINB) void kmeans_assign_top3_q1_v3_kernel(
    const TopQ1Table tbl, const __bf16* __restrict__ Ct, const float* __restrict__ chalf,
    int ntiles, int32_t* __restrict__ labels, FusedQ1Fin fin) {
  extern __shared__ __attribute__((aligned(16))) char smem[];
  const long b = hbmr_xcd_remap(blockIdx.x, gridDim.x);
  int lo = 0, hi = tbl.nsplit;
  while (hi - lo > 1) {
    const int mid = (lo + hi) >> 1;
    if (tbl.blk[mid] <= b) lo = mid; else hi = mid;
  }
  const int s = __builtin_amdgcn_readfirstlane(lo);
  const long o = tbl.off[s];
  fin.xnorm = tbl.xnorm[s];
  fin.xbn2 = tbl.xbn2[s];
  fin.xerr = tbl.xerr[s];
  fin.sidx = s;
  assign_tile_v3<D, F16>(tbl.X[s], tbl.off[s + 1] - o, Ct, chalf, ntiles, labels + o,
                         b - tbl.blk[s], smem, fin);
}

constexpr int kSweepPer = 8;
constexpr int kBoundHdr = 512;

struct ShiftTable {
  const float* ref[kMaxGroup];
};

__global__ __launch_bounds__(64) void kmeans_bound_shift_kernel(
    const ShiftTable tbl, const float* __restrict__ cen, int k, int d, float* __restrict__ shift,
    uint32_t* __restrict__ smax) {
  const int j = blockIdx.x, r = blockIdx.y;
  const float* a = cen + (size_t)j * d;
  const float* b = tbl.ref[r] + (size_t)j * d;
  double acc = 0.0;
  for (int i = threadIdx.x; i < d; i += 64) {
    const double e = (double)a[i] - (double)b[i];
    acc = fma(e, e, acc);
  }
#pragma unroll
  for (int off = 1; off < 64; off <<= 1) acc += __shfl_xor(acc, off);
  if (threadIdx.x == 0) {
    const float s = __double2float_ru(sqrt(acc) * (1.0 + 0x1p-40));
    shift[(size_t)r * k + j] = s;
    atomicMax(smax + r, __float_as_uint(s));
  }
}

__device__ __forceinline__ float sub_rd_pos(float a, float b) {
  const float t = a - b;
  if (!(t > 0x1p-100f)) return 0.f;
  const float bb = t - a;
  const float err = (a - (t - bb)) - (b + bb);
  return err < 0.f ? __uint_as_float(__float_as_uint(t) - 1u) : t;
}

struct SweepTable {
  int nsplit;
  const int32_t* g[kMaxGroup];
  float* gap[kMaxGroup];
  int rid[kMaxGroup];
  long n[kMaxGroup];
  long off[kMaxGroup];
  long blk[kMaxGroup + 1];
};

__global__ __launch_bounds__(256) void kmeans_bound_sweep_kernel(
    const SweepTable tbl, int k, const float* __restrict__ shift,
    const float* __restrict__ smax, int32_t* __restrict__ labels, uint32_t* __restrict__ cnt,
    uint32_t* __restrict__ idx) {
  const long b = blockIdx.x;
  int lo = 0, hi = tbl.nsplit;
  while (hi - lo > 1) {
    const int mid = (lo + hi) >> 1;
    if (tbl.blk[mid] <= b) lo = mid; else hi = mid;
  }
  const int s = __builtin_amdgcn_readfirstlane(lo);
  const int tid = threadIdx.x, lane = tid & 63, wave = tid >> 6;
  const long n = tbl.n[s], o = tbl.off[s];
  const int32_t* __restrict__ g = tbl.g[s];
  float* __restrict__ gap = tbl.gap[s];
  const float* __restrict__ sh = shift + (size_t)tbl.rid[s] * k;
  const float sm = gap ? smax[tbl.rid[s]] : 0.f;
  const long p0 = (b - tbl.blk[s]) * (256 * kSweepPer);
  __shared__ uint32_t wcnt[4][kSweepPer];
  __shared__ uint32_t base_s;
  bool list[kSweepPer];
  uint32_t rank[kSweepPer];
#pragma unroll
  for (int i = 0; i < kSweepPer; ++i) {
    const long p = p0 + i * 256 + tid;
    list[i] = false;
    if (p < n) {
      list[i] = true;
      if (gap) {
        const int32_t c = g[p];
        const float v =
            (uint32_t)c < (uint32_t)k ? sub_rd_pos(sub_rd_pos(gap[p], sh[c]), sm) : 0.f;
        if (v > 0.f) {
          list[i] = false;
          labels[o + p] = c;
          gap[p] = v;
        }
      }
    }
    const unsigned long long m = __ballot(list[i]);
    rank[i] = lane_rank(m);
    if (lane == 0) wcnt[wave][i] = (uint32_t)__popcll(m);
  }
  __syncthreads();
  if (tid == 0) {
    uint32_t tot = 0;
#pragma unroll
    for (int w = 0; w < 4; ++w)
#pragma unroll
      for (int i = 0; i < kSweepPer; ++i) {
        const uint32_t c = wcnt[w][i];
        wcnt[w][i] = tot;
        tot += c;
      }
    base_s = tot ? atomicAdd(cnt + s, tot) : 0u;
  }
  __syncthreads();
  uint32_t* out = idx + o + base_s;
#pragma unroll
  for (int i = 0; i < kSweepPer; ++i)
    if (list[i]) out[wcnt[wave][i] + rank[i]] = (uint32_t)(p0 + i * 256 + tid);
}

struct GapTable {
  float* gap[kMaxGroup];
};

template <int D, bool F16>
__global__ __launch_bounds__(256, HBMR_EXACT_MINB) void kmeans_assign_top3_q1_bounded_kernel(
    const TopQ1Table tbl, const GapTable gt, const __bf16* __restrict__ Ct,
    const float* __restrict__ chalf, int ntiles, int32_t* __restrict__ labels, FusedQ1Fin fin,
    const uint32_t* __restrict__ cnt, const uint32_t* __restrict__ idx,
    unsigned long long* __restrict__ skipped) {
  extern __shared__ __attribute__((aligned(16))) char smem[];
  if (blockIdx.x == 0 && threadIdx.x == 0 && skipped != nullptr) {
    unsigned long long sk = 0;
    for (int i = 0; i < tbl.nsplit; ++i)
      sk += (unsigned long long)(tbl.off[i + 1] - tbl.off[i]) - cnt[i];
    if (sk) atomicAdd(skipped, sk);
  }
  const long b = hbmr_xcd_remap(blockIdx.x, gridDim.x);
  int lo = 0, hi = tbl.nsplit;
  while (hi - lo > 1) {
    const int mid = (lo + hi) >> 1;
    if (tbl.blk[mid] <= b) lo = mid; else hi = mid;
  }
  const int s = __builtin_amdgcn_readfirstlane(lo);
  const long nl = (long)__builtin_amdgcn_readfirstlane(cnt[s]);
  const long lb = b - tbl.blk[s];
  if (lb * 256 >= nl) return;
  const long o = tbl.off[s];
  fin.xnorm = tbl.xnorm[s];
  fin.xbn2 = tbl.xbn2[s];
  fin.xerr = tbl.xerr[s];
  fin.sidx = s;
  fin.idx = idx + o;
  fin.gap = gt.gap[s];
  assign_tile_v3<D, F16, true>(tbl.X[s], nl, Ct, chalf, ntiles, labels + o, lb, smem, fin);
}

template <int NM>
__device__ __forceinline__ void load_row16(const float* __restrict__ r, int d, int sub,
                                           float (&v)[16 * NM]) {
#pragma unroll
  for (int m = 0; m < NM; ++m) {
#pragma unroll
    for (int h = 0; h < 4; ++h) {
      const int b = 128 * m + 32 * h + 4 * sub;
      const bool ok = b < d;
      const float4 a = *reinterpret_cast<const float4*>(r + (ok ? b : 0));
      float* o = v + 16 * m + 4 * h;
      o[0] = ok ? a.x : 0.f; o[1] = ok ? a.y : 0.f; o[2] = ok ? a.z : 0.f; o[3] = ok ? a.w : 0.f;
    }
  }
}

__device__ __forceinline__ float row_sum8f(float v) {
  v += __shfl_xor(v, 1);
  v += __shfl_xor(v, 2);
  v += __shfl_xor(v, 4);
  return v;
}

__device__ __forceinline__ double row_sum8(double v) {
  v += dpp_f64<0xB1>(v);
  v += dpp_f64<0x4E>(v);
  v += dpp_f64<0x141>(v);
  return v;
}

template <int NM>
__global__ __launch_bounds__(256) void kmeans_refine_q2_kernel(
    const RefineTable tbl, int d, int ldx, const float* __restrict__ C32, int k,
    const float* __restrict__ cmax, const float* __restrict__ cerrmax, double pack_rel,
    const uint32_t* __restrict__ qcount, const ExactQ1* __restrict__ q1, long cap1,
    uint32_t* __restrict__ q2count, ExactQ2* __restrict__ q2, long cap2,
    unsigned long long* __restrict__ sstats) {
  constexpr uint32_t kPerBlk = 4 * kQ2Per;
  constexpr uint32_t kBuf = 256;
  const int tid = threadIdx.x, lane = tid & 63, wave = tid >> 6;
  const int grp = lane / kQ2Lanes, sub = lane % kQ2Lanes;
  __shared__ ExactQ2 sbuf[kBuf];
  __shared__ uint32_t sn, sbase;
  __shared__ unsigned long long cnt[2];
  if (tid < 2) cnt[tid] = 0;
  if (tid == 0) sn = 0;
  __syncthreads();
  const double inflate = 1.0 + 0x1p-20;
  const double gam = (double)(d + 2) * 0x1p-23 * 1.01;
  const double cem = (double)cerrmax[0] * inflate;
  const double cm = (double)cmax[0] * inflate + cem;
  uint32_t c1[kQShards];
  uint32_t total = 0;
#pragma unroll
  for (int j = 0; j < kQShards; ++j) {
    c1[j] = qcount[j];
    total += c1[j];
  }
  const int shard = blockIdx.x % kQShards;
  const uint32_t stride = gridDim.x * kPerBlk;
  const uint32_t off = wave * kQ2Per + grp;
  auto flush = [&]() {
    if (tid == 0) {
      sbase = atomicAdd(q2count + shard, sn);
      cnt[1] += sn;
    }
    __syncthreads();
    const uint32_t m = sn;
    for (uint32_t i = tid; i < m; i += 256) q2[(long)shard * cap2 + sbase + i] = sbuf[i];
    __syncthreads();
    if (tid == 0) sn = 0;
    __syncthreads();
  };
  uint32_t bb = blockIdx.x * kPerBlk;
  ExactQ1 e;
  if (bb < total) e = q1[shard_slot(c1, cap1, min(bb + off, total - 1))];
  for (; bb < total; bb += stride) {
    const ExactQ1 q = e;
    const bool have = bb + off < total;
    const uint32_t nb = bb + stride;
    if (nb < total) e = q1[shard_slot(c1, cap1, min(nb + off, total - 1))];
    const bool t_real = q.t < k;
    const float* xr = tbl.x32[q.split] + (size_t)q.row * ldx;
    float xf[16 * NM], c0[16 * NM], c1r[16 * NM], c2[16 * NM];
    load_row16<NM>(xr, d, sub, xf);
    load_row16<NM>(C32 + (size_t)q.b * d, d, sub, c0);
    load_row16<NM>(C32 + (size_t)q.s * d, d, sub, c1r);
    load_row16<NM>(C32 + (size_t)(t_real ? q.t : q.b) * d, d, sub, c2);
    float f0 = 0.f, f1 = 0.f, f2 = 0.f;
#pragma unroll
    for (int i = 0; i < 16 * NM; ++i) {
      const float e0 = xf[i] - c0[i], e1 = xf[i] - c1r[i], e2 = xf[i] - c2[i];
      f0 = fmaf(e0, e0, f0);
      f1 = fmaf(e1, e1, f1);
      f2 = fmaf(e2, e2, f2);
    }
    f0 = row_sum8f(f0);
    f1 = row_sum8f(f1);
    f2 = row_sum8f(f2);
    const double rel = (double)(16 * NM + 8) * 0x1p-24 * 1.01, aeps = 0x1p-120;
    int w = q.b;
    double dw = f0;
    if ((double)f1 < dw || ((double)f1 == dw && q.s < w)) { w = q.s; dw = f1; }
    if (t_real && ((double)f2 < dw || ((double)f2 == dw && q.t < w))) { w = q.t; dw = f2; }
    const double whi = dw * (1.0 + rel) + aeps;
    auto beats = [&](double dj) { return dj * (1.0 - rel) - aeps > whi; };
    bool separated = isfinite(whi) &&
                     (w == q.b || beats(f0)) && (w == q.s || beats(f1)) &&
                     (!t_real || w == q.t || beats(f2));
    dw = whi;
    bool certified = !t_real && separated;
    if (t_real && separated) {
      const double xn = ((double)q.xn + (double)q.xe) * inflate;
      const double x2 = (double)q.x2;
      const double amax = ((double)q.xe + cem) * inflate;
      const double st = (double)q.sb - (double)q.m3;
      double et, dl_t;
      exact_bound(st, cm, xn, x2, amax, gam, pack_rel, et, dl_t);
      certified = 0.5 * (x2 - dw) - x2 * 0x1p-23 > st + et && dl_t >= 2.0 * amax;
    }
    if (have && sub == 0 && certified && w != q.b) {
      tbl.labels[q.split][q.row] = w;
      atomicAdd(&cnt[0], 1ull);
    }
    const bool spill = have && sub == 0 && !certified;
    const unsigned long long m = __ballot(spill);
    if (m) {
      uint32_t b2 = 0;
      if (lane == 0) b2 = atomicAdd(&sn, (uint32_t)__popcll(m));
      b2 = __shfl(b2, 0);
      if (spill) {
        ExactQ2 o;
        o.row = q.row;
        o.split = q.split;
        o.w = w;
        o.pad = 0;
        o.dw = dw;
        sbuf[b2 + lane_rank(m)] = o;
      }
    }
    __syncthreads();
    if (sn > kBuf - kPerBlk) flush();
  }
  __syncthreads();
  if (sn) flush();
  if (tid < 2 && cnt[tid]) atomicAdd(sstats + 4 * shard + 1 + tid, cnt[tid]);
}

template <int NM>
__global__ __launch_bounds__(256) void kmeans_refine_q3_kernel(
    const RefineTable tbl, int d, int ldx, const float* __restrict__ C32, int k,
    const int32_t* __restrict__ nbr_idx, const float* __restrict__ nbr_dist, int L,
    const uint32_t* __restrict__ q2count, const ExactQ2* __restrict__ q2, long cap2,
    unsigned long long* __restrict__ sstats, int nstats) {
  const int tid = threadIdx.x, lane = tid & 63;
  const int grp = lane / kRefineGroup, sub = lane % kRefineGroup;
  __shared__ unsigned long long cnt[3];
  if (tid < 3) cnt[tid] = 0;
  __syncthreads();
  uint32_t c2[kQShards];
  uint32_t total = 0;
#pragma unroll
  for (int j = 0; j < kQShards; ++j) {
    c2[j] = q2count[j];
    total += c2[j];
  }
  const uint32_t nwaves = gridDim.x * 4;
  const uint32_t gw = blockIdx.x * 4 + (tid >> 6);
  for (uint32_t base = gw * 4; base < total; base += nwaves * 4) {
    const uint32_t idx = base + grp;
    const bool have = idx < total;
    const ExactQ2 q = q2[shard_slot(c2, cap2, have ? idx : base)];
    int32_t* lab = tbl.labels[q.split];
    const int b0 = lab[q.row];
    double xv[8 * NM];
    {
      float xf[8 * NM];
      load_row8<NM>(tbl.x32[q.split] + (size_t)q.row * ldx, d, sub, xf);
#pragma unroll
      for (int i = 0; i < 8 * NM; ++i) xv[i] = (double)xf[i];
    }
    const int w0 = q.w;
    int w = w0;
    double dw;
    {
      const float* c0p[1] = {C32 + (size_t)w0 * d};
      double d0[1];
      rows_dist2<NM, 1>(xv, c0p, d, sub, d0);
      dw = d0[0];
    }
    const double r0 = sqrt(dw);
    bool done = false;
    const int32_t* ni = nbr_idx + (size_t)w0 * L;
    const float* nd = nbr_dist + (size_t)w0 * L;
    const float* cw0 = C32 + (size_t)w0 * d;
    int evals = 0;
    for (int jj = 0; jj < L; jj += kElkanStep) {
      const double lim = (r0 + sqrt(dw)) * (1.0 + 0x1p-40);
      if ((double)nd[jj] > lim) {
        done = true;
        break;
      }
      int jv[kElkanStep];
      const float* cp[kElkanStep];
#pragma unroll
      for (int v = 0; v < kElkanStep; ++v) {
        const bool ok = jj + v < L && (double)nd[jj + v] <= lim;
        jv[v] = ok ? ni[jj + v] : -1;
        cp[v] = ok ? C32 + (size_t)jv[v] * d : cw0;
      }
      double dj[kElkanStep];
      rows_dist2<NM, kElkanStep>(xv, cp, d, sub, dj);
      evals += kElkanStep;
#pragma unroll
      for (int v = 0; v < kElkanStep; ++v)
        if (jv[v] >= 0 && (dj[v] < dw || (dj[v] == dw && jv[v] < w))) { w = jv[v]; dw = dj[v]; }
    }
    const bool full = !done && L < k;
    if (full) {
      for (int j = 0; j < k; j += 4) {
        const float* cp[4];
#pragma unroll
        for (int v = 0; v < 4; ++v) cp[v] = C32 + (size_t)(j + v < k ? j + v : j) * d;
        double dj[4];
        rows_dist2<NM, 4>(xv, cp, d, sub, dj);
#pragma unroll
        for (int v = 0; v < 4; ++v)
          if (j + v < k && (dj[v] < dw || (dj[v] == dw && j + v < w))) { w = j + v; dw = dj[v]; }
      }
    }
    if (have && sub == 0) {
      atomicAdd(&cnt[1], (unsigned long long)evals);
      if (full) atomicAdd(&cnt[2], 1ull);
      if (w != b0) atomicAdd(&cnt[0], 1ull);
      lab[q.row] = w;
    }
  }
  __syncthreads();
  const int sh = blockIdx.x % (kQShards / 2);
  if (tid == 0 && cnt[0]) atomicAdd(sstats + 4 * sh + 1, cnt[0]);
  if (tid == 1 && cnt[1]) atomicAdd(sstats + 4 * sh + 3, cnt[1]);
  if (tid == 2 && cnt[2]) atomicAdd(sstats + 4 * (sh + kQShards / 2) + 3, cnt[2]);
}

__global__ void kmeans_refine_stats_kernel(const unsigned long long* __restrict__ ss,
                                           unsigned long long* __restrict__ stats, int nstats) {
  const int t = threadIdx.x;
  if (t >= 5 || (t >= 3 && nstats < 5)) return;
  unsigned long long v = 0;
  if (t < 3) {
    for (int j = 0; j < kQShards; ++j) v += ss[4 * j + t];
  } else {
    for (int j = 0; j < kQShards / 2; ++j) v += ss[4 * (j + (t - 3) * (kQShards / 2)) + 3];
  }
  if (v) stats[t] += v;
}

int refine_version() {
  static int v = 0;
  if (!v) {
    const char* e = getenv("HBMR_REFINE");
    v = (e && atoi(e) == 1) ? 1 : 2;
  }
  return v;
}

template <int D, bool F16>
int launch_assign_top3_grouped(int nsplit, const void* const* X, const long* n, const void* C,
                               const float* chalf, int k_pad, int32_t* labels, int32_t* cand,
                               float* scores, float* margin, hipStream_t st) {
  if constexpr (D > 128) {
    return (int)hipErrorNotSupported;
  } else {
    if (nsplit <= 0 || nsplit > kMaxGroup || k_pad % 32) return (int)hipErrorInvalidValue;
    SplitTable t;
    memset(&t, 0, sizeof(t));
    t.nsplit = nsplit;
    constexpr int pts = AssignV2<D>::WAVES * 2 * 32;
    long total = 0, nb = 0;
    for (int i = 0; i < nsplit; ++i) {
      if (n[i] < 0) return (int)hipErrorInvalidValue;
      t.X[i] = reinterpret_cast<const __bf16*>(X[i]);
      t.n[i] = n[i];
      t.off[i] = total;
      t.blk[i] = nb;
      total += n[i];
      nb += (n[i] + pts - 1) / pts;
    }
    t.blk[nsplit] = nb;
    if (nb == 0) return 0;
    if (nb > 0x7fffffffL) return (int)hipErrorInvalidValue;
    static const bool top3 = [] {
      const char* e = getenv("HBMR_EXACT_EPI");
      return e && strcmp(e, "top3") == 0;
    }();
    auto kern = top3 ? kmeans_assign_top3_grouped_v2_kernel<D, 2, F16, true>
                     : kmeans_assign_top3_grouped_v2_kernel<D, 2, F16, false>;
    hipLaunchKernelGGL(kern, dim3((unsigned)nb), dim3(AssignV2<D>::THREADS),
                       AssignV2<D>::LDS_BYTES, st, t, reinterpret_cast<const __bf16*>(C), chalf,
                       k_pad / 32, labels, cand, scores, margin, total);
    return (int)hipGetLastError();
  }
}

template <int D, bool F16>
int launch_assign_top3(const void* X, long n, const void* C, const float* chalf, int k_pad,
                       int32_t* labels, int32_t* cand, float* scores, float* margin,
                       hipStream_t st) {
  if (n <= 0) return 0;
  if (k_pad % kCK) return (int)hipErrorInvalidValue;
  if constexpr (D <= 128) {
    if (assign_version(D) == 2) {
      const int pts = AssignV2<D>::WAVES * 2 * 32;
      const long nblk = (n + pts - 1) / pts;
      if (nblk > 0x7fffffffL) return (int)hipErrorInvalidValue;
      static const bool top3 = [] {
        const char* e = getenv("HBMR_EXACT_EPI");
        return e && strcmp(e, "top3") == 0;
// ... 468 lines not shown
    default: return (int)hipErrorInvalidValue;
  }
#undef HBMR_TOP3G
}

int hbmr_kmeans_assign_top3_q1_grouped(int nsplit, const void* const* X, const long* n, int dp,
                                       int f16, const void* C, const void* Ct,
                                       const float* chalf, int k_pad,
                                       int32_t* labels, const float* const* xnorm,
                                       const float* const* xbn2, const float* const* xerr,
                                       int d, int k, const float* cnorm, const float* cmax,
                                       const float* cerr, const float* cerrmax, void* ws,
                                       long ws_bytes, const float* dcc, hipStream_t st) {
  if (nsplit <= 0 || nsplit > kMaxGroup || k_pad % 32 || k <= 0 || k_pad < k ||
      d > kRefineMaxDp || !labels || ((uintptr_t)ws & 255) || (dp != 64 && dp != 128))
    return (int)hipErrorInvalidValue;
  TopQ1Table t;
  memset(&t, 0, sizeof(t));
  t.nsplit = nsplit;
  constexpr int pts = 4 * 2 * 32;
  long total = 0, nb = 0;
  for (int i = 0; i < nsplit; ++i) {
    if (n[i] < 0 || n[i] > 0x7fffffffL) return (int)hipErrorInvalidValue;
    t.X[i] = reinterpret_cast<const __bf16*>(X[i]);
    t.xnorm[i] = xnorm[i];
    t.xbn2[i] = xbn2[i];
    t.xerr[i] = xerr[i];
    t.off[i] = total;
    t.blk[i] = nb;
    total += n[i];
    nb += ceil_div(n[i], pts);
  }
  t.off[nsplit] = total;
  t.blk[nsplit] = nb;
  const RefineLayout Ly = refine_layout(nsplit, n);
  if (ws_bytes < (long)Ly.bytes) return (int)hipErrorInvalidValue;
  char* w = static_cast<char*>(ws);
  HBMR_RETURN_IF_ERROR(hipMemsetAsync(w, 0, kHdrClear, st));
  if (nb == 0) return 0;
  if (nb > 0x7fffffffL) return (int)hipErrorInvalidValue;
  int tb = 0;
  while ((1 << tb) < k_pad / 32) ++tb;
  FusedQ1Fin fin;
  memset(&fin, 0, sizeof(fin));
  fin.k = k;
  const double inflate = 1.0 + 0x1p-20;
  fin.gam = (double)(d + 2) * 0x1p-23 * 1.01;
  fin.pack_rel = ldexp(1.0, 4 + tb - 23);
  fin.cnorm = cnorm;
  fin.cerr = cerr;
  fin.dcc = dcc;
  fin.qcount = reinterpret_cast<uint32_t*>(w);
  fin.q1 = reinterpret_cast<ExactQ1*>(w + Ly.off1);
  fin.cap1 = Ly.cap1;
  fin.stats = reinterpret_cast<unsigned long long*>(w + kStatsOff);
  fin.cmax_p = cmax;
  fin.cerrmax_p = cerrmax;
  (void)inflate;
  if (exact_kernel() == 3) {
    if (!Ct) return (int)hipErrorInvalidValue;
    auto kern = dp == 64 ? (f16 ? kmeans_assign_top3_q1_v3_kernel<64, true>
                                : kmeans_assign_top3_q1_v3_kernel<64, false>)
                         : (f16 ? kmeans_assign_top3_q1_v3_kernel<128, true>
                                : kmeans_assign_top3_q1_v3_kernel<128, false>);
    const size_t lds = dp == 64 ? AssignV2<64>::LDS_BYTES : AssignV2<128>::LDS_BYTES;
    hipLaunchKernelGGL(kern, dim3((unsigned)nb), dim3(256), lds, st, t,
                       reinterpret_cast<const __bf16*>(Ct), chalf, k_pad / 32, labels, fin);
    return (int)hipGetLastError();
  }
  auto kern = dp == 64 ? (f16 ? kmeans_assign_top3_q1_grouped_kernel<64, true>
                              : kmeans_assign_top3_q1_grouped_kernel<64, false>)
                       : (f16 ? kmeans_assign_top3_q1_grouped_kernel<128, true>
                              : kmeans_assign_top3_q1_grouped_kernel<128, false>);
  const size_t lds = dp == 64 ? AssignV2<64>::LDS_BYTES : AssignV2<128>::LDS_BYTES;
  hipLaunchKernelGGL(kern, dim3((unsigned)nb),
                     dim3(dp == 64 ? AssignV2<64>::THREADS : AssignV2<128>::THREADS), lds, st, t,
                     reinterpret_cast<const __bf16*>(C), chalf, k_pad / 32, labels, fin);
  return (int)hipGetLastError();
}

long hbmr_kmeans_bound_workspace_bytes(long total, int nsplit, int k) {
  if (total < 0 || nsplit <= 0 || nsplit > kMaxGroup || k <= 0) return -1;
  const size_t sh = ((size_t)nsplit * k * sizeof(float) + 255) & ~(size_t)255;
  return (long)(kBoundHdr + sh + (size_t)total * sizeof(uint32_t));
}

int hbmr_kmeans_assign_top3_q1_bounded(int nsplit, const void* const* X, const long* n, int dp,
                                       int f16, const void* Ct, const float* chalf, int k_pad,
                                       int32_t* labels, const float* const* xnorm,
                                       const float* const* xbn2, const float* const* xerr,
                                       int d, int k, const float* cnorm, const float* cmax,
                                       const float* cerr, const float* cerrmax, void* ws,
                                       long ws_bytes, const float* dcc,
                                       const int32_t* const* g, float* const* gap,
                                       const float* const* ref, const float* cen, void* bws,
                                       long bws_bytes, unsigned long long* skipped,
                                       hipStream_t st) {
  if (nsplit <= 0 || nsplit > kMaxGroup || k_pad % 32 || k <= 0 || k_pad < k || d <= 0 ||
      d > kRefineMaxDp || !labels || ((uintptr_t)ws & 255) || (dp != 64 && dp != 128) || !Ct ||
      !g || !gap || !ref || !cen || !bws || ((uintptr_t)bws & 255))
    return (int)hipErrorInvalidValue;
  TopQ1Table t;
  SweepTable sw;
  GapTable gt;
  ShiftTable sh;
  memset(&t, 0, sizeof(t));
  memset(&sw, 0, sizeof(sw));
  memset(&gt, 0, sizeof(gt));
  memset(&sh, 0, sizeof(sh));
  t.nsplit = sw.nsplit = nsplit;
  constexpr int pts = 4 * 2 * 32;
  long total = 0, nb = 0, nsb = 0;
  int nref = 0;
  for (int i = 0; i < nsplit; ++i) {
    if (n[i] < 0 || n[i] > 0x7fffffffL || !gap[i] || (ref[i] && !g[i]))
      return (int)hipErrorInvalidValue;
    t.X[i] = reinterpret_cast<const __bf16*>(X[i]);
    t.xnorm[i] = xnorm[i];
    t.xbn2[i] = xbn2[i];
    t.xerr[i] = xerr[i];
    t.off[i] = sw.off[i] = total;
    t.blk[i] = nb;
    sw.blk[i] = nsb;
    sw.n[i] = n[i];
    sw.g[i] = g[i];
    gt.gap[i] = gap[i];
    if (ref[i]) {
      int r = 0;
      while (r < nref && sh.ref[r] != ref[i]) ++r;
      if (r == nref) sh.ref[nref++] = ref[i];
      sw.rid[i] = r;
      sw.gap[i] = gap[i];
    }
    total += n[i];
    nb += ceil_div(n[i], pts);
    nsb += ceil_div(n[i], 256 * kSweepPer);
  }
  t.off[nsplit] = total;
  t.blk[nsplit] = nb;
  sw.blk[nsplit] = nsb;
  const RefineLayout Ly = refine_layout(nsplit, n);
  if (ws_bytes < (long)Ly.bytes ||
      bws_bytes < hbmr_kmeans_bound_workspace_bytes(total, nsplit, k))
    return (int)hipErrorInvalidValue;
  char* w = static_cast<char*>(ws);
  char* bw = static_cast<char*>(bws);
  HBMR_RETURN_IF_ERROR(hipMemsetAsync(w, 0, kHdrClear, st));
  if (nb == 0) return 0;
  if (nb > 0x7fffffffL) return (int)hipErrorInvalidValue;
  HBMR_RETURN_IF_ERROR(hipMemsetAsync(bw, 0, kBoundHdr, st));
  uint32_t* cnt = reinterpret_cast<uint32_t*>(bw);
  uint32_t* smax = cnt + kMaxGroup;
  float* shift = reinterpret_cast<float*>(bw + kBoundHdr);
  uint32_t* idx = reinterpret_cast<uint32_t*>(
      bw + kBoundHdr + (((size_t)nsplit * k * sizeof(float) + 255) & ~(size_t)255));
  if (nref > 0) {
    hipLaunchKernelGGL(kmeans_bound_shift_kernel, dim3((unsigned)k, (unsigned)nref), dim3(64), 0,
                       st, sh, cen, k, d, shift, smax);
    HBMR_RETURN_IF_ERROR(hipGetLastError());
  }
  hipLaunchKernelGGL(kmeans_bound_sweep_kernel, dim3((unsigned)nsb), dim3(256), 0, st, sw, k,
                     shift, reinterpret_cast<const float*>(smax), labels, cnt, idx);
  HBMR_RETURN_IF_ERROR(hipGetLastError());
  int tb = 0;
  while ((1 << tb) < k_pad / 32) ++tb;
  FusedQ1Fin fin;
  memset(&fin, 0, sizeof(fin));
  fin.k = k;
  fin.gam = (double)(d + 2) * 0x1p-23 * 1.01;
  fin.pack_rel = ldexp(1.0, 4 + tb - 23);
  fin.cnorm = cnorm;
  fin.cerr = cerr;
  fin.dcc = dcc;
  fin.qcount = reinterpret_cast<uint32_t*>(w);
  fin.q1 = reinterpret_cast<ExactQ1*>(w + Ly.off1);
  fin.cap1 = Ly.cap1;
  fin.stats = reinterpret_cast<unsigned long long*>(w + kStatsOff);
  fin.cmax_p = cmax;
  fin.cerrmax_p = cerrmax;
  auto kern = dp == 64 ? (f16 ? kmeans_assign_top3_q1_bounded_kernel<64, true>
                              : kmeans_assign_top3_q1_bounded_kernel<64, false>)
                       : (f16 ? kmeans_assign_top3_q1_bounded_kernel<128, true>
                              : kmeans_assign_top3_q1_bounded_kernel<128, false>);
  const size_t lds = dp == 64 ? AssignV2<64>::LDS_BYTES : AssignV2<128>::LDS_BYTES;
  hipLaunchKernelGGL(kern, dim3((unsigned)nb), dim3(256), lds, st, t, gt,
                     reinterpret_cast<const __bf16*>(Ct), chalf, k_pad / 32, labels, fin,
                     (const uint32_t*)cnt, (const uint32_t*)idx, skipped);
  return (int)hipGetLastError();
}

int hbmr_kmeans_refine_f32(const float* X32, long n, int d, int ldx, const float* xnorm,
                           const float* xbn2, const float* xerr, const float* C32, int k,
                           int k_pad, const float* cnorm, const float* cmax, const float* cerr,
                           const float* cerrmax, const int32_t* nbr_idx,
                           const float* nbr_dist, int L, int32_t* labels, const int32_t* cand,
                           const float* scores, const float* margin, unsigned long long* stats,
                           int nstats, hipStream_t st) {
  if (n <= 0) return 0;
  if (d > ldx || d > kRefineMaxDp || k <= 0 || k_pad < k || L < 1 || L > k)
    return (int)hipErrorInvalidValue;
  int tb = 0;
  while ((1 << tb) < k_pad / 32) ++tb;
  const double pack_rel = ldexp(1.0, 4 + tb - 23);
  const long blocks = (n + 255) / 256;
  const bool v2_ok = d % 8 == 0 && ldx % 4 == 0 && ((uintptr_t)X32 & 15) == 0 &&
                     ((uintptr_t)C32 & 15) == 0;
  if (v2_ok && refine_version() == 2) {
    auto kern = d <= 128 ? kmeans_refine_v2_kernel<1> : kmeans_refine_v2_kernel<2>;
    hipLaunchKernelGGL(kern, dim3((unsigned)blocks), dim3(256), 0, st, X32, n, d, ldx, xnorm,
                       xbn2, xerr, C32, k, cnorm, cmax, cerr, cerrmax, pack_rel, nbr_idx,
                       nbr_dist, L, labels, cand, scores, margin, stats, nstats);
    return (int)hipGetLastError();
  }
  hipLaunchKernelGGL(kmeans_refine_kernel, dim3((unsigned)blocks), dim3(256), 0, st, X32, n, d,
                     ldx, xnorm, xbn2, xerr, C32, k, cnorm, cmax, cerr, cerrmax, pack_rel,
                     nbr_idx, nbr_dist, L,
                     labels, cand, scores, margin, stats, nstats);
  return (int)hipGetLastError();
}


int hbmr_kmeans_exact_prep(const float* x, long n, int d, int ldx, int dp, int f16, void* x16,
                           float* xnorm, float* xn2, float* xerr, hipStream_t st) {
  if (n <= 0) return 0;
  if (d > ldx || d > dp || dp % 8 || !x16 || !xnorm || !xn2 || !xerr)
    return (int)hipErrorInvalidValue;
  const long blocks = (n + 15) / 16;
  if (blocks > 0x7fffffffL) return (int)hipErrorInvalidValue;
  hipLaunchKernelGGL(kmeans_exact_prep_kernel, dim3((unsigned)blocks), dim3(256), 0, st, x, n, d,
                     ldx, dp, f16, reinterpret_cast<uint16_t*>(x16), xnorm, xn2, xerr);
  return (int)hipGetLastError();
}

int hbmr_kmeans_set_exact_kernel(int v) {
  const int old = g_exact_kernel;
  g_exact_kernel = v == 2 || v == 3 ? v : -1;
  return old;
}

int hbmr_kmeans_get_exact_kernel(void) { return exact_kernel(); }

int hbmr_kmeans_image16_tiled(const void* c16, int k_pad, int dp, void* c16t, hipStream_t st) {
  if (k_pad <= 0 || k_pad % 32 || (dp != 64 && dp != 128) || !c16 || !c16t)
    return (int)hipErrorInvalidValue;
  const long pieces = (long)k_pad * dp / 8;
  hipLaunchKernelGGL(kmeans_image16_tiled_kernel, dim3((unsigned)((pieces + 255) / 256)),
                     dim3(256), 0, st, reinterpret_cast<const uint4*>(c16), k_pad, dp,
                     reinterpret_cast<uint4*>(c16t));
  return (int)hipGetLastError();
}

int hbmr_kmeans_image16(const float* cen, int k, int d, int dp, int k_pad, int f16, void* c16,
                        float* chalf, float* cnorm, float* cerr, float* maxima, hipStream_t st) {
  if (k <= 0 || k_pad < k || d > dp) return (int)hipErrorInvalidValue;
  HBMR_RETURN_IF_ERROR(hipMemsetAsync(maxima, 0, 2 * sizeof(float), st));
  hipLaunchKernelGGL(kmeans_image16_kernel, dim3((unsigned)k_pad), dim3(128), 0, st, cen, k, d,
                     dp, f16, reinterpret_cast<uint16_t*>(c16), chalf, cnorm, cerr,
                     reinterpret_cast<unsigned*>(maxima));
  return (int)hipGetLastError();
}


}

constexpr int kNbrThreads = 256;
constexpr int kNbrMaxD = 256;
constexpr int kNbrMaxK = 8192;

__global__ __launch_bounds__(kNbrThreads) void kmeans_centroid_nbr_kernel(
    const float* __restrict__ cen, int k, int d, int L, int kp2, double rel,
    int32_t* __restrict__ di, float* __restrict__ dv, float* __restrict__ pd) {
// ... 84 lines not shown
  hipLaunchKernelGGL(kmeans_centroid_nbr_kernel, dim3((unsigned)k), dim3(kNbrThreads), lds, st,
                     cen, k, d, L, kp2, rel, di, dv, pd);
  return (int)hipGetLastError();
}


long hbmr_kmeans_refine_batch_bytes(int nsplit, const long* ns) {
  if (nsplit <= 0 || nsplit > kMaxGroup) return -1;
  return (long)refine_layout(nsplit, ns).bytes;
}

int hbmr_kmeans_refine_batch_q1(int nsplit, const long* ns, int s, int d, int k, int k_pad,
                                const float* xnorm, const float* xbn2, const float* xerr,
                                const float* cnorm, const float* cmax, const float* cerr,
                                const float* cerrmax, const int32_t* labels, const int32_t* cand,
                                const float* scores, const float* margin,
                                unsigned long long* stats, void* ws, long ws_bytes, int reset,
                                const float* dcc, hipStream_t st) {
  if (nsplit <= 0 || nsplit > kMaxGroup || s < 0 || s >= nsplit || k <= 0 || k_pad < k ||
      d > kRefineMaxDp || ((uintptr_t)ws & 255))
    return (int)hipErrorInvalidValue;
  for (int i = 0; i < nsplit; ++i)
    if (ns[i] < 0 || ns[i] > 0x7fffffffL) return (int)hipErrorInvalidValue;
  const RefineLayout Ly = refine_layout(nsplit, ns);
  if (ws_bytes < (long)Ly.bytes) return (int)hipErrorInvalidValue;
  char* w = static_cast<char*>(ws);
  uint32_t* c1 = reinterpret_cast<uint32_t*>(w);
  if (reset) HBMR_RETURN_IF_ERROR(hipMemsetAsync(c1, 0, kHdrClear, st));
  const long n = ns[s];
  if (n == 0) return 0;
  int tb = 0;
  while ((1 << tb) < k_pad / 32) ++tb;
  const double pack_rel = ldexp(1.0, 4 + tb - 23);
  const long b1 = ceil_div(n, 256 * kQ1Per);
  hipLaunchKernelGGL(kmeans_refine_q1_kernel, dim3((unsigned)b1), dim3(256), 0, st, n, s, d, k,
                     xnorm, xbn2, xerr, cnorm, cmax, cerr, cerrmax, pack_rel, labels, cand,
                     scores, margin, c1, reinterpret_cast<ExactQ1*>(w + Ly.off1), Ly.cap1,
                     reinterpret_cast<unsigned long long*>(w + kStatsOff), dcc);
  return (int)hipGetLastError();
}

int hbmr_kmeans_refine_batch_q1g(int nsplit, const long* ns, int d, int k, int k_pad,
                                 const float* const* xnorm, const float* const* xbn2,
                                 const float* const* xerr, const float* cnorm, const float* cmax,
                                 const float* cerr, const float* cerrmax, const int32_t* labels,
                                 const int32_t* cand, const float* scores, const float* margin,
                                 void* ws, long ws_bytes, const float* dcc, hipStream_t st) {
  if (nsplit <= 0 || nsplit > kMaxGroup || k <= 0 || k_pad < k || d > kRefineMaxDp ||
      ((uintptr_t)ws & 255))
    return (int)hipErrorInvalidValue;
  Q1Table t;
  memset(&t, 0, sizeof(t));
  t.nsplit = nsplit;
  long total = 0, nb = 0;
  for (int i = 0; i < nsplit; ++i) {
    if (ns[i] < 0 || ns[i] > 0x7fffffffL) return (int)hipErrorInvalidValue;
    t.n[i] = ns[i];
    t.off[i] = total;
    t.blk[i] = nb;
    t.xnorm[i] = xnorm[i];
    t.xbn2[i] = xbn2[i];
    t.xerr[i] = xerr[i];
    total += ns[i];
    nb += ceil_div(ns[i], 256 * kQ1Per);
  }
  t.blk[nsplit] = nb;
  t.total = total;
  const RefineLayout Ly = refine_layout(nsplit, ns);
  if (ws_bytes < (long)Ly.bytes) return (int)hipErrorInvalidValue;
  char* w = static_cast<char*>(ws);
  uint32_t* c1 = reinterpret_cast<uint32_t*>(w);
  HBMR_RETURN_IF_ERROR(hipMemsetAsync(c1, 0, kHdrClear, st));
  if (nb == 0) return 0;
  int tb = 0;
  while ((1 << tb) < k_pad / 32) ++tb;
  const double pack_rel = ldexp(1.0, 4 + tb - 23);
  hipLaunchKernelGGL(kmeans_refine_q1_grouped_kernel, dim3((unsigned)nb), dim3(256), 0, st, t, d,
                     k, cnorm, cmax, cerr, cerrmax, pack_rel, labels, cand, scores, margin, c1,
                     reinterpret_cast<ExactQ1*>(w + Ly.off1), Ly.cap1,
                     reinterpret_cast<unsigned long long*>(w + kStatsOff), dcc);
  return (int)hipGetLastError();
}

int hbmr_kmeans_refine_batch_finish(int nsplit, const long* ns, const float* const* x32,
                                    int32_t* const* labels, int d, int ldx, const float* C32,
                                    int k, int k_pad, const float* cmax, const float* cerrmax,
                                    const int32_t* nbr_idx, const float* nbr_dist, int L,
                                    unsigned long long* stats, int nstats, void* ws,
                                    long ws_bytes, hipStream_t st) {
  if (nsplit <= 0 || nsplit > kMaxGroup || d > ldx || d > kRefineMaxDp || d % 8 || ldx % 4 ||
      k <= 0 || k_pad < k || L < 1 || L > k || nstats < 3 || ((uintptr_t)C32 & 15) ||
      ((uintptr_t)ws & 255))
    return (int)hipErrorInvalidValue;
  const RefineLayout Ly = refine_layout(nsplit, ns);
  if (ws_bytes < (long)Ly.bytes) return (int)hipErrorInvalidValue;
  RefineTable tbl;
  std::memset(&tbl, 0, sizeof(tbl));
  tbl.nsplit = nsplit;
  for (int i = 0; i < nsplit; ++i) {
    if ((uintptr_t)x32[i] & 15) return (int)hipErrorInvalidValue;
    tbl.x32[i] = x32[i];
    tbl.labels[i] = labels[i];
  }
  int tb = 0;
  while ((1 << tb) < k_pad / 32) ++tb;
  const double pack_rel = ldexp(1.0, 4 + tb - 23);
  char* w = static_cast<char*>(ws);
  uint32_t* c1 = reinterpret_cast<uint32_t*>(w);
  uint32_t* c2 = c1 + kQShards;
  const ExactQ1* q1 = reinterpret_cast<const ExactQ1*>(w + Ly.off1);
  ExactQ2* q2 = reinterpret_cast<ExactQ2*>(w + Ly.off2);
  unsigned long long* ss = reinterpret_cast<unsigned long long*>(w + kStatsOff);
  const unsigned g3 = std::max(1u, Ly.g2);
  if (d <= 128) {
    hipLaunchKernelGGL(kmeans_refine_q2_kernel<1>, dim3(Ly.g2), dim3(256), 0, st, tbl, d, ldx,
                       C32, k, cmax, cerrmax, pack_rel, c1, q1, Ly.cap1, c2, q2, Ly.cap2, ss);
    HBMR_RETURN_IF_ERROR(hipGetLastError());
    hipLaunchKernelGGL(kmeans_refine_q3_kernel<1>, dim3(g3), dim3(256), 0, st, tbl, d, ldx, C32,
                       k, nbr_idx, nbr_dist, L, c2, q2, Ly.cap2, ss, nstats);
  } else {
    hipLaunchKernelGGL(kmeans_refine_q2_kernel<2>, dim3(Ly.g2), dim3(256), 0, st, tbl, d, ldx,
                       C32, k, cmax, cerrmax, pack_rel, c1, q1, Ly.cap1, c2, q2, Ly.cap2, ss);
    HBMR_RETURN_IF_ERROR(hipGetLastError());
    hipLaunchKernelGGL(kmeans_refine_q3_kernel<2>, dim3(g3), dim3(256), 0, st, tbl, d, ldx, C32,
                       k, nbr_idx, nbr_dist, L, c2, q2, Ly.cap2, ss, nstats);
  }
  HBMR_RETURN_IF_ERROR(hipGetLastError());
  hipLaunchKernelGGL(kmeans_refine_stats_kernel, dim3(1), dim3(64), 0, st, ss, stats, nstats);
  return (int)hipGetLastError();
}

}
```

Baseline: 10410.

## Keep per-point candidate centroids so bounded exact assignment can settle points cheaply

Adds per-point state (two candidate centroid indices plus a residual bound) to the bounded exact K-Means path. Points whose stored bound fails are checked against only their few saved candidates in a new kernel instead of going through the full top-3 rescoring, and the refine kernels write the candidates back for the next iteration. The aim is to cut full-distance work for points near cluster boundaries across iterations. In exchange it costs extra device memory per point, an extra kernel launch, and more complex bound bookkeeping that has to stay exact.

```diff
diff --git a/hbmr/models/kmeans.py b/hbmr/models/kmeans.py
--- a/hbmr/models/kmeans.py
+++ b/hbmr/models/kmeans.py
@@ -29,6 +29,7 @@
 EXACT_MFMA_KEY = "hbmr.kmeans.exact.mfma"
 COMBINER_KEY = "hbmr.kmeans.combiner"
 BOUNDS_KEY = "hbmr.kmeans.exact.bounds"
+CANDIDATES_KEY = "hbmr.kmeans.exact.bounds.candidates"
 
 _M32 = 0xFFFFFFFF
 
@@ -288,7 +289,7 @@
     with _EXACT_LOCK:
         t = _EXACT_SKIPPED.get(key)
         if t is None:
-            t = _EXACT_SKIPPED[key] = torch.zeros(1, dtype=torch.int64, device=device)
+            t = _EXACT_SKIPPED[key] = torch.zeros(2, dtype=torch.int64, device=device)
         return t
 
 
@@ -311,6 +312,7 @@
         self.exact_dtype = torch.bfloat16 if (conf.get(EXACT_MFMA_KEY) or "f16").lower() in (
             "bf16", "bfloat16") else torch.float16
         self.bounds = conf.get_boolean(BOUNDS_KEY, True)
+        self.candidates = conf.get_boolean(CANDIDATES_KEY, True)
         self.combiner = (conf.get(COMBINER_KEY) or "delta").lower()
         if self.combiner not in ("delta", "sorted"):
             raise ValueError(f"{COMBINER_KEY} must be delta or sorted, not {self.combiner!r}")
@@ -569,11 +571,16 @@
             hb = [bases[i] for i in have]
             bounded = self.bounds and self.combiner == "delta" and km.bounds_supported(img)
             if bounded:
-                nogap = [b for b in hb if b.gap is None]
+                def held(b):
+                    return sum(t.numel() * t.element_size() for t in (b.gap, b.cand, b.rest)
+                               if t is not None)
+                grow = [(b, held(b)) for b in hb
+                        if b.gap is None or (self.candidates and b.cand is None)]
+                esk = _exact_skipped(self.cin, ctx.device)
                 km.assign_exact_batch([datas[i] for i in have], img, stats, lab, scratch,
-                                      stream=ctx.stream, bounds=hb,
-                                      skipped=_exact_skipped(self.cin, ctx.device))
-                grown = {id(b): b.gap.numel() * b.gap.element_size() for b in nogap}
+                                      stream=ctx.stream, bounds=hb, skipped=esk[0:1],
+                                      candidates=self.candidates, settled=esk[1:2])
+                grown = {id(b): held(b) - was for b, was in grow if held(b) > was}
             else:
                 km.assign_exact_batch([datas[i] for i in have], img, stats, lab, scratch,
                                       stream=ctx.stream)
@@ -705,11 +712,12 @@
             if est is not None:
                 vals += list(est.double().unbind(0))
             if esk is not None:
-                vals.append(esk[0].double())
+                vals += [esk[1].double(), esk[0].double()]
             got = torch.stack(vals).tolist()
             shift, npts = got[0], got[1]
             if esk is not None:
                 ctx.reporter.incrCounter("KMEANS", "EXACT_BOUND_SKIPPED_POINTS", int(got[-1]))
+                ctx.reporter.incrCounter("KMEANS", "EXACT_BOUND_CANDIDATE_POINTS", int(got[-2]))
             if est is not None:
                 for name, v in zip(("EXACT_FLAGGED_POINTS", "EXACT_RELABELLED_POINTS",
                                     "EXACT_NEIGHBOUR_SCANS"), got[2:5]):
diff --git a/hbmr/ops/_lib.py b/hbmr/ops/_lib.py
--- a/hbmr/ops/_lib.py
+++ b/hbmr/ops/_lib.py
@@ -44,6 +44,16 @@
                                                    c_void_p, c_long, c_void_p,
                                                    c_void_p, c_void_p, c_void_p, c_void_p,
                                                    c_void_p, c_long, c_void_p, c_void_p]),
+    "hbmr_kmeans_bound_lists_offset": (c_long, [c_int, c_int]),
+    "hbmr_kmeans_assign_top3_q1_bounded_cand": (c_int, [c_int, c_void_p, c_void_p, c_int, c_int,
+                                                        c_void_p, c_void_p, c_int, c_void_p,
+                                                        c_void_p, c_void_p, c_void_p, c_int,
+                                                        c_int, c_void_p, c_void_p, c_void_p,
+                                                        c_void_p, c_void_p, c_long, c_void_p,
+                                                        c_void_p, c_void_p, c_void_p, c_void_p,
+                                                        c_void_p, c_long, c_void_p,
+                                                        c_void_p, c_int, c_void_p, c_void_p,
+                                                        c_void_p, c_void_p]),
     "hbmr_kmeans_centroid_nbr": (c_int, [c_void_p, c_int, c_int, c_int, c_void_p, c_void_p,
                                          c_void_p, c_void_p]),
     "hbmr_kmeans_image16": (c_int, [c_void_p, c_int, c_int, c_int, c_int, c_int, c_void_p,
@@ -73,6 +83,11 @@
                                                 c_int, c_void_p, c_int, c_int, c_void_p,
                                                 c_void_p, c_void_p, c_void_p, c_int, c_void_p,
                                                 c_int, c_void_p, c_long, c_void_p]),
+    "hbmr_kmeans_refine_batch_finish_cand": (c_int, [c_int, c_void_p, c_void_p, c_void_p, c_int,
+                                                     c_int, c_void_p, c_int, c_int, c_void_p,
+                                                     c_void_p, c_void_p, c_void_p, c_int,
+                                                     c_void_p, c_int, c_void_p, c_long, c_void_p,
+                                                     c_void_p, c_void_p]),
     "hbmr_kmeans_accum_workspace_bytes": (c_long, [c_long, c_int]),
     "hbmr_kmeans_batch_workspace_bytes": (c_long, [c_long, c_int, c_int]),
     "hbmr_kmeans_map_batch": (c_int, [c_int, c_void_p, c_void_p, c_int, c_void_p, c_void_p, c_int,
diff --git a/hbmr/ops/kmeans.py b/hbmr/ops/kmeans.py
--- a/hbmr/ops/kmeans.py
+++ b/hbmr/ops/kmeans.py
@@ -342,7 +342,7 @@
             _ptr(self.ws), self.ws.numel(), int(i == 0), _ptr(self.pd), self.st)
         _lib.check(rc, "hbmr_kmeans_refine_batch_q1")
 
-    def finish(self):
+    def finish(self, bases=None):
         B = len(self.splits)
         img = self.img
         _, cmax, _, cemax = self.norms
@@ -350,6 +350,16 @@
         xs = (ctypes.c_void_p * B)(*[sp.x32.data_ptr() for sp in self.splits])
         ls = (ctypes.c_void_p * B)(*[(lp.value if isinstance(lp, ctypes.c_void_p) else lp)
                                      for lp in self.labels])
+        if bases is not None:
+            P = ctypes.c_void_p * B
+            rc = self.lib.hbmr_kmeans_refine_batch_finish_cand(
+                B, self.ns, xs, ls, img.d, self.splits[0].x32.shape[1], _ptr(img.cen), img.k,
+                img.k_pad, _ptr(cmax), _ptr(cemax), _ptr(ni), _ptr(nd), L, _ptr(self.stats),
+                self.stats.numel(), _ptr(self.ws), self.ws.numel(),
+                P(*[b.cand.data_ptr() for b in bases]), P(*[b.rest.data_ptr() for b in bases]),
+                self.st)
+            _lib.check(rc, "hbmr_kmeans_refine_batch_finish_cand")
+            return
         rc = self.lib.hbmr_kmeans_refine_batch_finish(
             B, self.ns, xs, ls, img.d, self.splits[0].x32.shape[1], _ptr(img.cen), img.k,
             img.k_pad, _ptr(cmax), _ptr(cemax), _ptr(ni), _ptr(nd), L, _ptr(self.stats),
@@ -406,7 +416,8 @@
 
 def assign_exact_batch(splits: list, img: CentroidImage, stats: torch.Tensor, out: torch.Tensor,
                        scratch: dict | None = None, stream=None, bounds: list | None = None,
-                       skipped: torch.Tensor | None = None) -> None:
+                       skipped: torch.Tensor | None = None, candidates: bool = True,
+                       settled: torch.Tensor | None = None) -> None:
     if not splits:
         return
     if bounds is not None and (len(bounds) != len(splits) or not bounds_supported(img)):
@@ -455,7 +466,7 @@
             off += _exact_group(group, img, stats, base + 4 * off, c16, ch, (cn, cmax, ce, cemax),
                                 dt, scratch, stream, lib, st,
                                 None if bounds is None else bounds[g0:g0 + MAX_REFINE_BATCH],
-                                skipped, newref)
+                                skipped, newref, candidates, settled)
             continue
         rb = _RefineBatch(group, img, stats, scratch, stream) if REFINE_VERSION >= 3 else None
         for i, sp in enumerate(group):
@@ -483,7 +494,7 @@
 
 
 def _bounded_group(group, bases, img, labels_ptr, ch, norms, dt, scratch, stream, lib, st, rb,
-                   skipped, newref):
+                   skipped, newref, candidates=False, settled=None):
     B = len(group)
     ns = [sp.shape[0] for sp in group]
     N = sum(ns)
@@ -499,12 +510,20 @@
         for b in bases:
             if b.gap is None:
                 b.gap, b.ref = torch.empty(b.g.numel(), dtype=torch.float32, device=dev), None
+            if not candidates:
+                b.cand = b.rest = None
+            elif b.cand is None or b.rest is None:
+                b.cand = torch.full((b.g.numel(), 2), -1, dtype=torch.int32, device=dev)
+                b.rest = torch.zeros(b.g.numel(), dtype=torch.float32, device=dev)
         for b, n in zip(bases, ns):
+            if candidates and (b.cand.numel() != 2 * n or b.rest.numel() != n or
+                               not b.cand.is_contiguous()):
+                raise ValueError("bounds: candidate state does not match its split")
             if b.g.numel() != n or b.gap.numel() != n or \
                     (b.ref is not None and (tuple(b.ref.shape) != tuple(img.cen.shape) or
                                             not b.ref.is_contiguous())):
                 raise ValueError("bounds: baseline does not match its split / the centroids")
-            for t in (b.g, b.gap, b.ref):
+            for t in (b.g, b.gap, b.ref, b.cand, b.rest):
                 if t is not None:
                     base = t._base if t._base is not None else t
                     blocks[id(base)] = base
@@ -519,7 +538,7 @@
     refs = [b.ref for b in bases]
     for b in bases:
         b.ref = b.pending = None
-    rc = lib.hbmr_kmeans_assign_top3_q1_bounded(
+    args = (
         B, P(*[sp.xb.data_ptr() for sp in group]), (ctypes.c_long * B)(*ns), img.dp,
         int(dt == torch.float16), _ptr(img.image16_tiled(dt)), _ptr(ch), img.k_pad, labels_ptr,
         P(*[sp.xnorm.data_ptr() for sp in group]), P(*[sp.xbn2.data_ptr() for sp in group]),
@@ -527,14 +546,36 @@
         _ptr(cemax), _ptr(rb.ws), rb.ws.numel(), _ptr(rb.pd),
         P(*[b.g.data_ptr() for b in bases]), P(*[b.gap.data_ptr() for b in bases]),
         P(*[None if r is None else r.data_ptr() for r in refs]), _ptr(img.cen),
-        _ptr(bws), bws.numel(), _ptr(skipped), st)
-    _lib.check(rc, "hbmr_kmeans_assign_top3_q1_bounded")
+        _ptr(bws), bws.numel(), _ptr(skipped))
+    if candidates:
+        rc = lib.hbmr_kmeans_assign_top3_q1_bounded_cand(
+            *args, P(*[sp.x32.data_ptr() for sp in group]), group[0].x32.shape[1],
+            P(*[b.cand.data_ptr() for b in bases]), P(*[b.rest.data_ptr() for b in bases]),
+            _ptr(settled), st)
+        _lib.check(rc, "hbmr_kmeans_assign_top3_q1_bounded_cand")
+    else:
+        rc = lib.hbmr_kmeans_assign_top3_q1_bounded(*args, st)
+        _lib.check(rc, "hbmr_kmeans_assign_top3_q1_bounded")
     for b in bases:
         b.pending = newref
 
 
+def bounded_lists(bws: torch.Tensor, ns: list, k: int):
+    B, total = len(ns), sum(ns)
+    words = bws.view(torch.int32)
+    cnt = words[:B].tolist()
+    ccnt = words[128:128 + B].tolist()
+    o = int(_lib.load().hbmr_kmeans_bound_lists_offset(B, k)) // 4
+    full, cand, at = [], [], 0
+    for i, n in enumerate(ns):
+        full.append(words[o + at:o + at + cnt[i]].long())
+        cand.append(words[o + total + at:o + total + at + ccnt[i]].long())
+        at += n
+    return full, cand
+
+
 def _exact_group(group, img, stats, labels_ptr, c16, ch, norms, dt, scratch, stream, lib, st,
-                 bases=None, skipped=None, newref=None):
+                 bases=None, skipped=None, newref=None, candidates=False, settled=None):
     B = len(group)
     ns = [sp.shape[0] for sp in group]
     N = sum(ns)
@@ -547,12 +588,12 @@
         if TRACE.on:
             TRACE.instant("kmeans.top3_launch", n=B)
         _bounded_group(group, bases, img, labels_ptr, ch, norms, dt, scratch, stream, lib, st, rb,
-                       skipped, newref)
+                       skipped, newref, candidates, settled)
         o = 0
         for i in range(B):
             rb.labels[i] = labels_ptr + 4 * o
             o += ns[i]
-        rb.finish()
+        rb.finish(bases if candidates else None)
         return N
     if FUSED_Q1 and img.dp <= 128:
         rb = _RefineBatch(group, img, stats, scratch, stream)
@@ -640,11 +681,13 @@
 
 
 class Baseline:
-    __slots__ = ("g", "S0", "N0", "event", "stream", "data_ptr", "n", "gap", "ref", "pending")
+    __slots__ = ("g", "S0", "N0", "event", "stream", "data_ptr", "n", "gap", "ref", "pending",
+                 "cand", "rest")
 
     def __init__(self, g, S0, N0, data_ptr, n):
         self.g, self.S0, self.N0 = g, S0, N0
         self.gap = self.ref = self.pending = None
+        self.cand = self.rest = None
         self.event = None
         self.stream = None
         self.data_ptr, self.n = data_ptr, n
diff --git a/native/include/hbmr/hbmr.h b/native/include/hbmr/hbmr.h
--- a/native/include/hbmr/hbmr.h
+++ b/native/include/hbmr/hbmr.h
@@ -59,6 +59,16 @@
                                        const float* const* ref, const float* cen, void* bws,
                                        long bws_bytes, unsigned long long* skipped,
                                        hipStream_t st);
+long hbmr_kmeans_bound_lists_offset(int nsplit, int k);
+int hbmr_kmeans_assign_top3_q1_bounded_cand(
+    int nsplit, const void* const* X, const long* n, int dp, int f16, const void* Ct,
+    const float* chalf, int k_pad, int32_t* labels, const float* const* xnorm,
+    const float* const* xbn2, const float* const* xerr, int d, int k, const float* cnorm,
+    const float* cmax, const float* cerr, const float* cerrmax, void* ws, long ws_bytes,
+    const float* dcc, const int32_t* const* g, float* const* gap, const float* const* ref,
+    const float* cen, void* bws, long bws_bytes, unsigned long long* skipped,
+    const float* const* x32, int ldx, int32_t* const* cand, float* const* rest,
+    unsigned long long* settled, hipStream_t st);
 int hbmr_kmeans_assign_top3_grouped(int nsplit, const void* const* X, const long* n, int dp,
                                     int f16, const void* C, const float* chalf, int k_pad,
                                     int32_t* labels, int32_t* cand, float* scores, float* margin,
@@ -83,6 +93,14 @@
                                     const int32_t* nbr_idx, const float* nbr_dist, int L,
                                     unsigned long long* stats, int nstats, void* ws,
                                     long ws_bytes, hipStream_t st);
+int hbmr_kmeans_refine_batch_finish_cand(int nsplit, const long* ns, const float* const* x32,
+                                         int32_t* const* labels, int d, int ldx,
+                                         const float* C32, int k, int k_pad, const float* cmax,
+                                         const float* cerrmax, const int32_t* nbr_idx,
+                                         const float* nbr_dist, int L, unsigned long long* stats,
+                                         int nstats, void* ws, long ws_bytes,
+                                         int32_t* const* cand, float* const* rest,
+                                         hipStream_t st);
 int hbmr_kmeans_update(const long long* sums, const long long* counts, int fx_shift, int k, int d,
                        int dp, int k_pad, float* cen, void* cbf, float* chalf, float* shift2,
                        hipStream_t st);
diff --git a/native/kernels/kmeans.hip b/native/kernels/kmeans.hip
--- a/native/kernels/kmeans.hip
+++ b/native/kernels/kmeans.hip
@@ -2059,6 +2059,10 @@
   const float* x32[kMaxGroup];
   int32_t* labels[kMaxGroup];
 };
+struct RefineState {
+  int32_t* cand[kMaxGroup];
+  float* rest[kMaxGroup];
+};
 
 __host__ __device__ inline long ceil_div(long a, long b) { return (a + b - 1) / b; }
 
@@ -2300,6 +2304,8 @@
   unsigned long long* stats;
   const uint32_t* idx;
   float* gap;
+  int32_t* cand;
+  float* rest;
 
   template <class AM, int PB, bool BND = false>
   __device__ __forceinline__ void operator()(const AM (&am)[PB], int h, long p0, int col, long n,
@@ -2361,6 +2367,24 @@
           flag[pb] = q.s < k && q1_certify<true>(q, m2, cnorm[q.b], cerr[q.b], k, gam, cm, cem,
                                                  pack_rel, cnorm, cerr, dcc, gp);
           gap[row] = gp;
+          if (cand != nullptr) {
+            const bool s_real = q.s < k;
+            const bool t_real = s_real && q.t < k && q.t != q.b;
+            float rs = 0.f;
+            if (t_real) {
+              const double x2 = (double)q.x2;
+              const double st = (double)q.sb - (double)q.m3;
+              double et, dl_t;
+              exact_bound(st, cm, ((double)q.xn + (double)q.xe) * inflate, x2,
+                          ((double)q.xe + cem) * inflate, gam, pack_rel, et, dl_t);
+              const double dlow = x2 * (1.0 - 0x1p-22) - 2.0 * (st + et);
+              if (dl_t >= 2.0 * ((double)q.xe + cem) * inflate && dlow > 0.0)
+                rs = fmaxf(0.f, __double2float_rd(sqrt(dlow) * (1.0 - 0x1p-30) * (1.0 - 0x1p-30)));
+            }
+            *reinterpret_cast<int2*>(cand + 2 * (size_t)row) =
+                make_int2(s_real ? q.s : -1, t_real ? q.t : -1);
+            rest[row] = rs;
+          }
         } else {
           flag[pb] = q.s < k && q1_flagged(q, m2, cnorm[q.b], cerr[q.b], k, gam, cm, cem,
                                            pack_rel, cnorm, cerr, dcc);
@@ -2585,7 +2609,7 @@
 }
 
 constexpr int kSweepPer = 8;
-constexpr int kBoundHdr = 512;
+constexpr int kBoundHdr = 2048;
 
 struct ShiftTable {
   const float* ref[kMaxGroup];
@@ -2623,6 +2647,7 @@
   int nsplit;
   const int32_t* g[kMaxGroup];
   float* gap[kMaxGroup];
+  float* rest[kMaxGroup];
   int rid[kMaxGroup];
   long n[kMaxGroup];
   long off[kMaxGroup];
@@ -2632,7 +2657,7 @@
 __global__ __launch_bounds__(256) void kmeans_bound_sweep_kernel(
     const SweepTable tbl, int k, const float* __restrict__ shift,
     const float* __restrict__ smax, int32_t* __restrict__ labels, uint32_t* __restrict__ cnt,
-    uint32_t* __restrict__ idx) {
+    uint32_t* __restrict__ idx, uint32_t* __restrict__ ccnt, uint32_t* __restrict__ cidx) {
   const long b = blockIdx.x;
   int lo = 0, hi = tbl.nsplit;
   while (hi - lo > 1) {
@@ -2644,56 +2669,93 @@
   const long n = tbl.n[s], o = tbl.off[s];
   const int32_t* __restrict__ g = tbl.g[s];
   float* __restrict__ gap = tbl.gap[s];
+  float* __restrict__ rest = gap ? tbl.rest[s] : nullptr;
   const float* __restrict__ sh = shift + (size_t)tbl.rid[s] * k;
   const float sm = gap ? smax[tbl.rid[s]] : 0.f;
   const long p0 = (b - tbl.blk[s]) * (256 * kSweepPer);
-  __shared__ uint32_t wcnt[4][kSweepPer];
-  __shared__ uint32_t base_s;
-  bool list[kSweepPer];
+  __shared__ uint32_t wcnt[2][4][kSweepPer];
+  __shared__ uint32_t base_s[2];
+  bool list[kSweepPer], clist[kSweepPer];
   uint32_t rank[kSweepPer];
 #pragma unroll
   for (int i = 0; i < kSweepPer; ++i) {
     const long p = p0 + i * 256 + tid;
-    list[i] = false;
+    list[i] = clist[i] = false;
     if (p < n) {
       list[i] = true;
       if (gap) {
         const int32_t c = g[p];
-        const float v =
-            (uint32_t)c < (uint32_t)k ? sub_rd_pos(sub_rd_pos(gap[p], sh[c]), sm) : 0.f;
+        const bool cok = (uint32_t)c < (uint32_t)k;
+        const float v = cok ? sub_rd_pos(sub_rd_pos(gap[p], sh[c]), sm) : 0.f;
+        float r = 0.f;
+        if (rest) {
+          const float r0 = rest[p];
+          r = r0 > 0.f ? sub_rd_pos(r0, sm) : 0.f;
+          if (r != r0) rest[p] = r;
+        }
         if (v > 0.f) {
           list[i] = false;
           labels[o + p] = c;
           gap[p] = v;
+        } else if (cok && r > 0.f) {
+          list[i] = false;
+          clist[i] = true;
         }
       }
     }
     const unsigned long long m = __ballot(list[i]);
-    rank[i] = lane_rank(m);
-    if (lane == 0) wcnt[wave][i] = (uint32_t)__popcll(m);
+    const unsigned long long mc = __ballot(clist[i]);
+    rank[i] = lane_rank(clist[i] ? mc : m);
+    if (lane == 0) {
+      wcnt[0][wave][i] = (uint32_t)__popcll(m);
+      wcnt[1][wave][i] = (uint32_t)__popcll(mc);
+    }
   }
   __syncthreads();
-  if (tid == 0) {
+  if (tid < 2) {
     uint32_t tot = 0;
 #pragma unroll
     for (int w = 0; w < 4; ++w)
 #pragma unroll
       for (int i = 0; i < kSweepPer; ++i) {
-        const uint32_t c = wcnt[w][i];
-        wcnt[w][i] = tot;
+        const uint32_t c = wcnt[tid][w][i];
+        wcnt[tid][w][i] = tot;
         tot += c;
       }
-    base_s = tot ? atomicAdd(cnt + s, tot) : 0u;
+    base_s[tid] = tot ? atomicAdd((tid ? ccnt : cnt) + s, tot) : 0u;
   }
   __syncthreads();
-  uint32_t* out = idx + o + base_s;
-#pragma unroll
-  for (int i = 0; i < kSweepPer; ++i)
-    if (list[i]) out[wcnt[wave][i] + rank[i]] = (uint32_t)(p0 + i * 256 + tid);
+  uint32_t* out = idx + o + base_s[0];
+  uint32_t* cout = cidx + o + base_s[1];
+#pragma unroll
+  for (int i = 0; i < kSweepPer; ++i) {
+    if (list[i]) out[wcnt[0][wave][i] + rank[i]] = (uint32_t)(p0 + i * 256 + tid);
+    if (clist[i]) cout[wcnt[1][wave][i] + rank[i]] = (uint32_t)(p0 + i * 256 + tid);
+  }
 }
 
 struct GapTable {
   float* gap[kMaxGroup];
+};
+
+struct CandState {
+  unsigned long long settled;
+  unsigned long long pad;
+  int32_t* cand[kMaxGroup];
+  float* rest[kMaxGroup];
+};
+constexpr int kCandCntOff = 512;
+constexpr int kCandStateOff = 768;
+static_assert(kCandStateOff + sizeof(CandState) <= kBoundHdr, "bounded workspace header");
+
+struct CandTable {
+  int nsplit;
+  const float* x32[kMaxGroup];
+  const int32_t* g[kMaxGroup];
+  int32_t* cand[kMaxGroup];
+  float* rest[kMaxGroup];
+  float* gap[kMaxGroup];
+  long off[kMaxGroup + 1];
 };
 
 template <int D, bool F16>
@@ -2701,13 +2763,18 @@
     const TopQ1Table tbl, const GapTable gt, const __bf16* __restrict__ Ct,
     const float* __restrict__ chalf, int ntiles, int32_t* __restrict__ labels, FusedQ1Fin fin,
     const uint32_t* __restrict__ cnt, const uint32_t* __restrict__ idx,
-    unsigned long long* __restrict__ skipped) {
+    unsigned long long* __restrict__ skipped, const CandState* __restrict__ cst,
+    unsigned long long* __restrict__ settled) {
   extern __shared__ __attribute__((aligned(16))) char smem[];
-  if (blockIdx.x == 0 && threadIdx.x == 0 && skipped != nullptr) {
-    unsigned long long sk = 0;
-    for (int i = 0; i < tbl.nsplit; ++i)
-      sk += (unsigned long long)(tbl.off[i + 1] - tbl.off[i]) - cnt[i];
-    if (sk) atomicAdd(skipped, sk);
+  if (blockIdx.x == 0 && threadIdx.x == 0) {
+    const unsigned long long se = cst ? cst->settled : 0ull;
+    if (skipped != nullptr) {
+      unsigned long long sk = 0;
+      for (int i = 0; i < tbl.nsplit; ++i)
+        sk += (unsigned long long)(tbl.off[i + 1] - tbl.off[i]) - cnt[i];
+      if (sk - se) atomicAdd(skipped, sk - se);
+    }
+    if (settled != nullptr && se) atomicAdd(settled, se);
   }
   const long b = hbmr_xcd_remap(blockIdx.x, gridDim.x);
   int lo = 0, hi = tbl.nsplit;
@@ -2726,6 +2793,10 @@
   fin.sidx = s;
   fin.idx = idx + o;
   fin.gap = gt.gap[s];
+  if (cst != nullptr) {
+    fin.cand = cst->cand[s];
+    fin.rest = cst->rest[s];
+  }
   assign_tile_v3<D, F16, true>(tbl.X[s], nl, Ct, chalf, ntiles, labels + o, lb, smem, fin);
 }
 
@@ -2765,7 +2836,7 @@
     const float* __restrict__ cmax, const float* __restrict__ cerrmax, double pack_rel,
     const uint32_t* __restrict__ qcount, const ExactQ1* __restrict__ q1, long cap1,
     uint32_t* __restrict__ q2count, ExactQ2* __restrict__ q2, long cap2,
-    unsigned long long* __restrict__ sstats) {
+    unsigned long long* __restrict__ sstats, const RefineState rst) {
   constexpr uint32_t kPerBlk = 4 * kQ2Per;
   constexpr uint32_t kBuf = 256;
   const int tid = threadIdx.x, lane = tid & 63, wave = tid >> 6;
@@ -2852,6 +2923,12 @@
     if (have && sub == 0 && certified && w != q.b) {
       tbl.labels[q.split][q.row] = w;
       atomicAdd(&cnt[0], 1ull);
+      int32_t* cd = rst.cand[q.split];
+      if (cd != nullptr) {
+        const int t2 = t_real && q.t != q.b ? q.t : -1;
+        *reinterpret_cast<int2*>(cd + 2 * (size_t)q.row) =
+            w == q.s ? make_int2(q.b, t2) : make_int2(q.s, q.b);
+      }
     }
     const bool spill = have && sub == 0 && !certified;
     const unsigned long long m = __ballot(spill);
@@ -2877,12 +2954,168 @@
   if (tid < 2 && cnt[tid]) atomicAdd(sstats + 4 * shard + 1 + tid, cnt[tid]);
 }
 
+struct CandEntry {
+  uint32_t row;
+  int s, g, c0, c1;
+  float rest;
+};
+
+template <int NM>
+__global__ __launch_bounds__(256) void kmeans_bound_cand_kernel(
+    const CandTable tbl, int d, int ldx, const float* __restrict__ C32, int k,
+    int32_t* __restrict__ labels, uint32_t* __restrict__ cnt, uint32_t* __restrict__ idx,
+    const uint32_t* __restrict__ ccnt, const uint32_t* __restrict__ cidx,
+    CandState* __restrict__ cst) {
+  constexpr uint32_t kPerBlk = 4 * kQ2Per;
+  constexpr uint32_t kBuf = 256;
+  const int tid = threadIdx.x, lane = tid & 63, wave = tid >> 6;
+  const int grp = lane / kQ2Lanes, sub = lane % kQ2Lanes;
+  __shared__ uint32_t pre[kMaxGroup + 1];
+  __shared__ uint32_t scnt[kMaxGroup], sbase[kMaxGroup];
+  __shared__ uint32_t srow[kBuf], sslot[kBuf];
+  __shared__ uint32_t sn;
+  __shared__ unsigned long long nset;
+  if (blockIdx.x == 0 && tid < kMaxGroup) {
+    cst->cand[tid] = tbl.cand[tid];
+    cst->rest[tid] = tbl.rest[tid];
+  }
+  if (tid < kMaxGroup) {
+    const uint32_t c = tid < tbl.nsplit ? ccnt[tid] : 0u;
+    uint32_t inc = c;
+#pragma unroll
+    for (int o = 1; o < kMaxGroup; o <<= 1) {
+      const uint32_t u = __shfl_up(inc, o);
+      if (lane >= o) inc += u;
+    }
+    pre[tid + 1] = inc;
+    scnt[tid] = 0;
+    if (tid == 0) {
+      pre[0] = 0;
+      sn = 0;
+      nset = 0;
+    }
+  }
+  __syncthreads();
+  const uint32_t total = pre[kMaxGroup];
+  const uint32_t stride = gridDim.x * kPerBlk;
+  const uint32_t off = wave * kQ2Per + grp;
+  auto fetch = [&](uint32_t i) {
+    int lo = 0, hi = tbl.nsplit;
+    while (hi - lo > 1) {
+      const int mid = (lo + hi) >> 1;
+      if (pre[mid] <= i) lo = mid; else hi = mid;
+    }
+    CandEntry e;
+    e.s = lo;
+    e.row = cidx[tbl.off[lo] + (i - pre[lo])];
+    e.g = tbl.g[lo][e.row];
+    const int2 c = *reinterpret_cast<const int2*>(tbl.cand[lo] + 2 * (size_t)e.row);
+    e.c0 = c.x;
+    e.c1 = c.y;
+    e.rest = tbl.rest[lo][e.row];
+    return e;
+  };
+  auto flush = [&]() {
+    if (tid < kMaxGroup && scnt[tid]) sbase[tid] = atomicAdd(cnt + tid, scnt[tid]);
+    __syncthreads();
+    const uint32_t m = sn;
+    for (uint32_t i = tid; i < m; i += 256) {
+      const uint32_t s = sslot[i] >> 16, pos = sslot[i] & 0xffffu;
+      idx[tbl.off[s] + sbase[s] + pos] = srow[i];
+    }
+    __syncthreads();
+    if (tid < kMaxGroup) scnt[tid] = 0;
+    if (tid == 0) sn = 0;
+    __syncthreads();
+  };
+  uint32_t bb = blockIdx.x * kPerBlk;
+  CandEntry e;
+  if (bb < total) e = fetch(min(bb + off, total - 1));
+  for (; bb < total; bb += stride) {
+    const CandEntry q = e;
+    const bool have = bb + off < total;
+    const uint32_t nb = bb + stride;
+    if (nb < total) e = fetch(min(nb + off, total - 1));
+    const bool two = q.c1 >= 0;
+    const bool valid = (uint32_t)q.g < (uint32_t)k && (uint32_t)q.c0 < (uint32_t)k &&
+                       (!two || (uint32_t)q.c1 < (uint32_t)k) && q.c0 != q.g && q.c1 != q.g &&
+                       q.c0 != q.c1;
+    const int g0 = valid ? q.g : 0;
+    const float* xr = tbl.x32[q.s] + (size_t)q.row * ldx;
+    float xf[16 * NM], c0[16 * NM], c1r[16 * NM], c2[16 * NM];
+    load_row16<NM>(xr, d, sub, xf);
+    load_row16<NM>(C32 + (size_t)g0 * d, d, sub, c0);
+    load_row16<NM>(C32 + (size_t)(valid ? q.c0 : 0) * d, d, sub, c1r);
+    load_row16<NM>(C32 + (size_t)(valid && two ? q.c1 : g0) * d, d, sub, c2);
+    float f0 = 0.f, f1 = 0.f, f2 = 0.f;
+#pragma unroll
+    for (int i = 0; i < 16 * NM; ++i) {
+      const float e0 = xf[i] - c0[i], e1 = xf[i] - c1r[i], e2 = xf[i] - c2[i];
+      f0 = fmaf(e0, e0, f0);
+      f1 = fmaf(e1, e1, f1);
+      f2 = fmaf(e2, e2, f2);
+    }
+    f0 = row_sum8f(f0);
+    f1 = row_sum8f(f1);
+    f2 = row_sum8f(f2);
+    const double rel = (double)(16 * NM + 8) * 0x1p-24 * 1.01, aeps = 0x1p-120;
+    int w = q.g;
+    double dw = f0;
+    if ((double)f1 < dw) { w = q.c0; dw = f1; }
+    if (two && (double)f2 < dw) { w = q.c1; dw = f2; }
+    const double whi = dw * (1.0 + rel) + aeps;
+    auto low = [&](double dj) { return dj * (1.0 - rel) - aeps; };
+    double olo = 0x1p1000;
+    if (w != q.g) olo = fmin(olo, low(f0));
+    if (w != q.c0) olo = fmin(olo, low(f1));
+    if (two && w != q.c1) olo = fmin(olo, low(f2));
+    const float up = __double2float_ru(sqrt(whi) * (1.0 + 0x1p-40));
+    const bool settle = have && valid && isfinite(whi) && olo > whi && up < q.rest;
+    if (settle && sub == 0) {
+      const float lo2 = __double2float_rd(sqrt(olo) * (1.0 - 0x1p-40));
+      labels[tbl.off[q.s] + q.row] = w;
+      tbl.gap[q.s][q.row] = sub_rd_pos(fminf(lo2, q.rest), up);
+      if (w != q.g)
+        *reinterpret_cast<int2*>(tbl.cand[q.s] + 2 * (size_t)q.row) =
+            w == q.c0 ? make_int2(q.g, q.c1) : make_int2(q.c0, q.g);
+    }
+    const unsigned long long ms = __ballot(settle && sub == 0);
+    if (lane == 0 && ms) atomicAdd(&nset, (unsigned long long)__popcll(ms));
+    if (have && sub == 0 && !settle) {
+      const uint32_t pos = atomicAdd(&scnt[q.s], 1u);
+      const uint32_t slot = atomicAdd(&sn, 1u);
+      srow[slot] = q.row;
+      sslot[slot] = ((uint32_t)q.s << 16) | pos;
+    }
+    __syncthreads();
+    if (sn > kBuf - kPerBlk) flush();
+  }
+  __syncthreads();
+  if (sn) flush();
+  if (tid == 0 && nset) atomicAdd(&cst->settled, nset);
+}
+
+__device__ __forceinline__ void best4_insert(double (&bd)[4], int (&bi)[4], double v, int j) {
+  if (j == bi[0] || j == bi[1] || j == bi[2] || j == bi[3]) return;
+#pragma unroll
+  for (int i = 0; i < 4; ++i) {
+    if (v < bd[i] || (v == bd[i] && (uint32_t)j < (uint32_t)bi[i])) {
+      const double tv = bd[i];
+      const int tj = bi[i];
+      bd[i] = v;
+      bi[i] = j;
+      v = tv;
+      j = tj;
+    }
+  }
+}
+
 template <int NM>
 __global__ __launch_bounds__(256) void kmeans_refine_q3_kernel(
     const RefineTable tbl, int d, int ldx, const float* __restrict__ C32, int k,
     const int32_t* __restrict__ nbr_idx, const float* __restrict__ nbr_dist, int L,
     const uint32_t* __restrict__ q2count, const ExactQ2* __restrict__ q2, long cap2,
-    unsigned long long* __restrict__ sstats, int nstats) {
+    unsigned long long* __restrict__ sstats, int nstats, const RefineState rst) {
   const int tid = threadIdx.x, lane = tid & 63;
   const int grp = lane / kRefineGroup, sub = lane % kRefineGroup;
   __shared__ unsigned long long cnt[3];
@@ -2921,6 +3154,9 @@
     }
     const double r0 = sqrt(dw);
     bool done = false;
+    double bd[4] = {dw, 0x1p1000, 0x1p1000, 0x1p1000};
+    int bi[4] = {w0, -1, -1, -1};
+    float ustop = __builtin_inff();
     const int32_t* ni = nbr_idx + (size_t)w0 * L;
     const float* nd = nbr_dist + (size_t)w0 * L;
     const float* cw0 = C32 + (size_t)w0 * d;
@@ -2929,6 +3165,7 @@
       const double lim = (r0 + sqrt(dw)) * (1.0 + 0x1p-40);
       if ((double)nd[jj] > lim) {
         done = true;
+        ustop = fminf(ustop, nd[jj]);
         break;
       }
       int jv[kElkanStep];
@@ -2936,6 +3173,7 @@
 #pragma unroll
       for (int v = 0; v < kElkanStep; ++v) {
         const bool ok = jj + v < L && (double)nd[jj + v] <= lim;
+        if (!ok && jj + v < L) ustop = fminf(ustop, nd[jj + v]);
         jv[v] = ok ? ni[jj + v] : -1;
         cp[v] = ok ? C32 + (size_t)jv[v] * d : cw0;
       }
@@ -2944,7 +3182,10 @@
       evals += kElkanStep;
 #pragma unroll
       for (int v = 0; v < kElkanStep; ++v)
-        if (jv[v] >= 0 && (dj[v] < dw || (dj[v] == dw && jv[v] < w))) { w = jv[v]; dw = dj[v]; }
+        if (jv[v] >= 0) {
+          if (dj[v] < dw || (dj[v] == dw && jv[v] < w)) { w = jv[v]; dw = dj[v]; }
+          best4_insert(bd, bi, dj[v], jv[v]);
+        }
     }
     const bool full = !done && L < k;
     if (full) {
@@ -2956,7 +3197,10 @@
         rows_dist2<NM, 4>(xv, cp, d, sub, dj);
 #pragma unroll
         for (int v = 0; v < 4; ++v)
-          if (j + v < k && (dj[v] < dw || (dj[v] == dw && j + v < w))) { w = j + v; dw = dj[v]; }
+          if (j + v < k) {
+            if (dj[v] < dw || (dj[v] == dw && j + v < w)) { w = j + v; dw = dj[v]; }
+            best4_insert(bd, bi, dj[v], j + v);
+          }
       }
     }
     if (have && sub == 0) {
@@ -2964,6 +3208,18 @@
       if (full) atomicAdd(&cnt[2], 1ull);
       if (w != b0) atomicAdd(&cnt[0], 1ull);
       lab[q.row] = w;
+      int32_t* cd = rst.cand[q.split];
+      if (cd != nullptr) {
+        double lo = bi[3] >= 0 ? sqrt(bd[3]) * (1.0 - 0x1p-30) : 0x1p1000;
+        if (!full && ustop < __builtin_inff())
+          lo = fmin(lo, ((double)ustop - r0 * (1.0 + 0x1p-40)) * (1.0 - 0x1p-30));
+        float rs = 0.f;
+        if (bi[0] == w && lo > 0.0)
+          rs = lo >= 0x1p127 ? 0x1p127f : __double2float_rd(lo);
+        *reinterpret_cast<int2*>(cd + 2 * (size_t)q.row) =
+            rs > 0.f ? make_int2(bi[1], bi[2]) : make_int2(-1, -1);
+        rst.rest[q.split][q.row] = rs;
+      }
     }
   }
   __syncthreads();
@@ -3598,10 +3854,16 @@
 long hbmr_kmeans_bound_workspace_bytes(long total, int nsplit, int k) {
   if (total < 0 || nsplit <= 0 || nsplit > kMaxGroup || k <= 0) return -1;
   const size_t sh = ((size_t)nsplit * k * sizeof(float) + 255) & ~(size_t)255;
-  return (long)(kBoundHdr + sh + (size_t)total * sizeof(uint32_t));
-}
-
-int hbmr_kmeans_assign_top3_q1_bounded(int nsplit, const void* const* X, const long* n, int dp,
+  return (long)(kBoundHdr + sh + 2 * (size_t)total * sizeof(uint32_t));
+}
+
+long hbmr_kmeans_bound_lists_offset(int nsplit, int k) {
+  if (nsplit <= 0 || nsplit > kMaxGroup || k <= 0) return -1;
+  static_assert(kCandCntOff == 128 * 4, "candidate list counts");
+  return (long)(kBoundHdr + (((size_t)nsplit * k * sizeof(float) + 255) & ~(size_t)255));
+}
+
+static int assign_top3_q1_bounded_impl(int nsplit, const void* const* X, const long* n, int dp,
                                        int f16, const void* Ct, const float* chalf, int k_pad,
                                        int32_t* labels, const float* const* xnorm,
                                        const float* const* xbn2, const float* const* xerr,
@@ -3611,7 +3873,15 @@
                                        const int32_t* const* g, float* const* gap,
                                        const float* const* ref, const float* cen, void* bws,
                                        long bws_bytes, unsigned long long* skipped,
+                                       const float* const* x32, int ldx, int32_t* const* cand,
+                                       float* const* rest, unsigned long long* settled,
                                        hipStream_t st) {
+  const bool cs = cand != nullptr;
+  if (cs && (!x32 || !rest || d > ldx || d % 8 || ldx % 4 || ((uintptr_t)cen & 15)))
+    return (int)hipErrorInvalidValue;
+  CandTable ct;
+  memset(&ct, 0, sizeof(ct));
+  ct.nsplit = nsplit;
   if (nsplit <= 0 || nsplit > kMaxGroup || k_pad % 32 || k <= 0 || k_pad < k || d <= 0 ||
       d > kRefineMaxDp || !labels || ((uintptr_t)ws & 255) || (dp != 64 && dp != 128) || !Ct ||
       !g || !gap || !ref || !cen || !bws || ((uintptr_t)bws & 255))
@@ -3641,6 +3911,17 @@
     sw.n[i] = n[i];
     sw.g[i] = g[i];
     gt.gap[i] = gap[i];
+    if (cs) {
+      if (!cand[i] || !rest[i] || !x32[i] || ((uintptr_t)x32[i] & 15) || ((uintptr_t)cand[i] & 7))
+        return (int)hipErrorInvalidValue;
+      ct.x32[i] = x32[i];
+      ct.g[i] = g[i];
+      ct.cand[i] = cand[i];
+      ct.rest[i] = rest[i];
+      ct.gap[i] = gap[i];
+      ct.off[i] = total;
+      if (ref[i]) sw.rest[i] = rest[i];
+    }
     if (ref[i]) {
       int r = 0;
       while (r < nref && sh.ref[r] != ref[i]) ++r;
@@ -3652,7 +3933,7 @@
     nb += ceil_div(n[i], pts);
     nsb += ceil_div(n[i], 256 * kSweepPer);
   }
-  t.off[nsplit] = total;
+  t.off[nsplit] = ct.off[nsplit] = total;
   t.blk[nsplit] = nb;
   sw.blk[nsplit] = nsb;
   const RefineLayout Ly = refine_layout(nsplit, n);
@@ -3670,14 +3951,28 @@
   float* shift = reinterpret_cast<float*>(bw + kBoundHdr);
   uint32_t* idx = reinterpret_cast<uint32_t*>(
       bw + kBoundHdr + (((size_t)nsplit * k * sizeof(float) + 255) & ~(size_t)255));
+  uint32_t* ccnt = reinterpret_cast<uint32_t*>(bw + kCandCntOff);
+  uint32_t* cidx = idx + total;
+  CandState* cst = reinterpret_cast<CandState*>(bw + kCandStateOff);
   if (nref > 0) {
     hipLaunchKernelGGL(kmeans_bound_shift_kernel, dim3((unsigned)k, (unsigned)nref), dim3(64), 0,
                        st, sh, cen, k, d, shift, smax);
     HBMR_RETURN_IF_ERROR(hipGetLastError());
   }
   hipLaunchKernelGGL(kmeans_bound_sweep_kernel, dim3((unsigned)nsb), dim3(256), 0, st, sw, k,
-                     shift, reinterpret_cast<const float*>(smax), labels, cnt, idx);
+                     shift, reinterpret_cast<const float*>(smax), labels, cnt, idx, ccnt, cidx);
   HBMR_RETURN_IF_ERROR(hipGetLastError());
+  if (cs) {
+    const unsigned gc = (unsigned)std::max<long>(
+        1, nref > 0 ? std::min<long>(refine_grid(), ceil_div(total, 4 * kQ2Per)) : 1);
+    if (d <= 128)
+      hipLaunchKernelGGL(kmeans_bound_cand_kernel<1>, dim3(gc), dim3(256), 0, st, ct, d, ldx, cen,
+                         k, labels, cnt, idx, (const uint32_t*)ccnt, (const uint32_t*)cidx, cst);
+    else
+      hipLaunchKernelGGL(kmeans_bound_cand_kernel<2>, dim3(gc), dim3(256), 0, st, ct, d, ldx, cen,
+                         k, labels, cnt, idx, (const uint32_t*)ccnt, (const uint32_t*)cidx, cst);
+    HBMR_RETURN_IF_ERROR(hipGetLastError());
+  }
   int tb = 0;
   while ((1 << tb) < k_pad / 32) ++tb;
   FusedQ1Fin fin;
@@ -3701,8 +3996,42 @@
   const size_t lds = dp == 64 ? AssignV2<64>::LDS_BYTES : AssignV2<128>::LDS_BYTES;
   hipLaunchKernelGGL(kern, dim3((unsigned)nb), dim3(256), lds, st, t, gt,
                      reinterpret_cast<const __bf16*>(Ct), chalf, k_pad / 32, labels, fin,
-                     (const uint32_t*)cnt, (const uint32_t*)idx, skipped);
+                     (const uint32_t*)cnt, (const uint32_t*)idx, skipped,
+                     cs ? (const CandState*)cst : nullptr, cs ? settled : nullptr);
   return (int)hipGetLastError();
+}
+
+int hbmr_kmeans_assign_top3_q1_bounded(int nsplit, const void* const* X, const long* n, int dp,
+                                       int f16, const void* Ct, const float* chalf, int k_pad,
+                                       int32_t* labels, const float* const* xnorm,
+                                       const float* const* xbn2, const float* const* xerr,
+                                       int d, int k, const float* cnorm, const float* cmax,
+                                       const float* cerr, const float* cerrmax, void* ws,
+                                       long ws_bytes, const float* dcc,
+                                       const int32_t* const* g, float* const* gap,
+                                       const float* const* ref, const float* cen, void* bws,
+                                       long bws_bytes, unsigned long long* skipped,
+                                       hipStream_t st) {
+  return assign_top3_q1_bounded_impl(nsplit, X, n, dp, f16, Ct, chalf, k_pad, labels, xnorm, xbn2,
+                                     xerr, d, k, cnorm, cmax, cerr, cerrmax, ws, ws_bytes, dcc, g,
+                                     gap, ref, cen, bws, bws_bytes, skipped, nullptr, 0, nullptr,
+                                     nullptr, nullptr, st);
+}
+
+int hbmr_kmeans_assign_top3_q1_bounded_cand(
+    int nsplit, const void* const* X, const long* n, int dp, int f16, const void* Ct,
+    const float* chalf, int k_pad, int32_t* labels, const float* const* xnorm,
+    const float* const* xbn2, const float* const* xerr, int d, int k, const float* cnorm,
+    const float* cmax, const float* cerr, const float* cerrmax, void* ws, long ws_bytes,
+    const float* dcc, const int32_t* const* g, float* const* gap, const float* const* ref,
+    const float* cen, void* bws, long bws_bytes, unsigned long long* skipped,
+    const float* const* x32, int ldx, int32_t* const* cand, float* const* rest,
+    unsigned long long* settled, hipStream_t st) {
+  if (!x32 || !cand || !rest) return (int)hipErrorInvalidValue;
+  return assign_top3_q1_bounded_impl(nsplit, X, n, dp, f16, Ct, chalf, k_pad, labels, xnorm, xbn2,
+                                     xerr, d, k, cnorm, cmax, cerr, cerrmax, ws, ws_bytes, dcc, g,
+                                     gap, ref, cen, bws, bws_bytes, skipped, x32, ldx, cand, rest,
+                                     settled, st);
 }
 
 int hbmr_kmeans_refine_f32(const float* X32, long n, int d, int ldx, const float* xnorm,
@@ -3953,12 +4282,23 @@
   return (int)hipGetLastError();
 }
 
-int hbmr_kmeans_refine_batch_finish(int nsplit, const long* ns, const float* const* x32,
+static int refine_batch_finish_impl(int nsplit, const long* ns, const float* const* x32,
                                     int32_t* const* labels, int d, int ldx, const float* C32,
                                     int k, int k_pad, const float* cmax, const float* cerrmax,
                                     const int32_t* nbr_idx, const float* nbr_dist, int L,
                                     unsigned long long* stats, int nstats, void* ws,
-                                    long ws_bytes, hipStream_t st) {
+                                    long ws_bytes, int32_t* const* cand, float* const* rest,
+                                    hipStream_t st) {
+  RefineState rst;
+  std::memset(&rst, 0, sizeof(rst));
+  if (cand != nullptr) {
+    if (!rest || nsplit <= 0 || nsplit > kMaxGroup) return (int)hipErrorInvalidValue;
+    for (int i = 0; i < nsplit; ++i) {
+      if (!cand[i] || !rest[i] || ((uintptr_t)cand[i] & 7)) return (int)hipErrorInvalidValue;
+      rst.cand[i] = cand[i];
+      rst.rest[i] = rest[i];
+    }
+  }
   if (nsplit <= 0 || nsplit > kMaxGroup || d > ldx || d > kRefineMaxDp || d % 8 || ldx % 4 ||
       k <= 0 || k_pad < k || L < 1 || L > k || nstats < 3 || ((uintptr_t)C32 & 15) ||
       ((uintptr_t)ws & 255))
@@ -3985,20 +4325,45 @@
   const unsigned g3 = std::max(1u, Ly.g2);
   if (d <= 128) {
     hipLaunchKernelGGL(kmeans_refine_q2_kernel<1>, dim3(Ly.g2), dim3(256), 0, st, tbl, d, ldx,
-                       C32, k, cmax, cerrmax, pack_rel, c1, q1, Ly.cap1, c2, q2, Ly.cap2, ss);
+                       C32, k, cmax, cerrmax, pack_rel, c1, q1, Ly.cap1, c2, q2, Ly.cap2, ss, rst);
     HBMR_RETURN_IF_ERROR(hipGetLastError());
     hipLaunchKernelGGL(kmeans_refine_q3_kernel<1>, dim3(g3), dim3(256), 0, st, tbl, d, ldx, C32,
-                       k, nbr_idx, nbr_dist, L, c2, q2, Ly.cap2, ss, nstats);
+                       k, nbr_idx, nbr_dist, L, c2, q2, Ly.cap2, ss, nstats, rst);
   } else {
     hipLaunchKernelGGL(kmeans_refine_q2_kernel<2>, dim3(Ly.g2), dim3(256), 0, st, tbl, d, ldx,
-                       C32, k, cmax, cerrmax, pack_rel, c1, q1, Ly.cap1, c2, q2, Ly.cap2, ss);
+                       C32, k, cmax, cerrmax, pack_rel, c1, q1, Ly.cap1, c2, q2, Ly.cap2, ss, rst);
     HBMR_RETURN_IF_ERROR(hipGetLastError());
     hipLaunchKernelGGL(kmeans_refine_q3_kernel<2>, dim3(g3), dim3(256), 0, st, tbl, d, ldx, C32,
-                       k, nbr_idx, nbr_dist, L, c2, q2, Ly.cap2, ss, nstats);
+                       k, nbr_idx, nbr_dist, L, c2, q2, Ly.cap2, ss, nstats, rst);
   }
   HBMR_RETURN_IF_ERROR(hipGetLastError());
   hipLaunchKernelGGL(kmeans_refine_stats_kernel, dim3(1), dim3(64), 0, st, ss, stats, nstats);
   return (int)hipGetLastError();
 }
 
-}
+int hbmr_kmeans_refine_batch_finish(int nsplit, const long* ns, const float* const* x32,
+                                    int32_t* const* labels, int d, int ldx, const float* C32,
+                                    int k, int k_pad, const float* cmax, const float* cerrmax,
+                                    const int32_t* nbr_idx, const float* nbr_dist, int L,
+                                    unsigned long long* stats, int nstats, void* ws,
+                                    long ws_bytes, hipStream_t st) {
+  return refine_batch_finish_impl(nsplit, ns, x32, labels, d, ldx, C32, k, k_pad, cmax, cerrmax,
+                                  nbr_idx, nbr_dist, L, stats, nstats, ws, ws_bytes, nullptr,
+                                  nullptr, st);
+}
+
+int hbmr_kmeans_refine_batch_finish_cand(int nsplit, const long* ns, const float* const* x32,
+                                         int32_t* const* labels, int d, int ldx,
+                                         const float* C32, int k, int k_pad, const float* cmax,
+                                         const float* cerrmax, const int32_t* nbr_idx,
+                                         const float* nbr_dist, int L, unsigned long long* stats,
+                                         int nstats, void* ws, long ws_bytes,
+                                         int32_t* const* cand, float* const* rest,
+                                         hipStream_t st) {
+  if (!cand || !rest) return (int)hipErrorInvalidValue;
+  return refine_batch_finish_impl(nsplit, ns, x32, labels, d, ldx, C32, k, k_pad, cmax, cerrmax,
+                                  nbr_idx, nbr_dist, L, stats, nstats, ws, ws_bytes, cand, rest,
+                                  st);
+}
+
+}
```

Measured after the change: 9497. -8.8%, worse.
